# zju3dv/disprcnn

Hardware: AMD Instinct MI355X
Metric: ROI cost-volumes/sec (112x112x48) (higher is better)
Workload: dtype f32 (every convolution of the regressor, the three 32->1 heads included: split-f16 -- each fp32 value carried as hi + lo fp16, 3 f16-MFMA products per fp32 product, f32 accumulate; fp32-class error, tests/test_hip_s16.py.  Head gather and soft-argmin: f32 VALU); 1 GPU; Config A: per ROI pair, features [32,28,28]x2 -> concat cost volume [64,12,28,28] (folded into the first 3D layer's loads, never written) -> 3D stacked-hourglass regressor -> trilinear x4 + softmax + soft-argmin -> disparity [112,112]; maxdisp=48, mindisp=0, parallelism=roi-shard x1 (no collective), weights=closed-form synthetic (disprcnn_amd.utils.synth), BN stats calibrated fixture

## Files before the change

disprcnn_amd/_lib.py:

```python
import ctypes as C
import os

import torch

_HERE = os.path.dirname(os.path.abspath(__file__))
LIB_PATH = os.path.join(_HERE, "csrc", "libdisprcnn_hip.so")

DRC_MAX_CLASSES = 8


class DrcTapClass(C.Structure):
    _fields_ = [("nd", C.c_int32), ("nh", C.c_int32), ("nw", C.c_int32),
                ("dd0", C.c_int32), ("dh0", C.c_int32), ("dw0", C.c_int32),
                ("sd", C.c_int32), ("sh", C.c_int32), ("sw", C.c_int32),
                ("wbase", C.c_int32), ("wsd", C.c_int32), ("wsh", C.c_int32), ("wsw", C.c_int32),
                ("out_off_d", C.c_int32), ("out_off_h", C.c_int32), ("out_off_w", C.c_int32)]


class DrcTapconvParams(C.Structure):
    _fields_ = [("x", C.c_void_p), ("w", C.c_void_p), ("scale", C.c_void_p), ("shift", C.c_void_p),
                ("res", C.c_void_p), ("y", C.c_void_p),
                ("x_n_stride", C.c_int64), ("x_cb_stride", C.c_int64), ("x_d_stride", C.c_int64), ("x_h_stride", C.c_int64),
                ("y_n_stride", C.c_int64), ("y_cb_stride", C.c_int64), ("y_d_stride", C.c_int64), ("y_h_stride", C.c_int64),
                ("y_off0", C.c_int64),
                ("r_n_stride", C.c_int64), ("r_cb_stride", C.c_int64), ("r_d_stride", C.c_int64), ("r_h_stride", C.c_int64),
                ("r_off0", C.c_int64),
                ("N", C.c_int32), ("OD", C.c_int32), ("OH", C.c_int32), ("OW", C.c_int32),
                ("in_mul", C.c_int32), ("out_mul", C.c_int32), ("cb_in", C.c_int32), ("cout_pad", C.c_int32),
                ("R", C.c_int32), ("WT", C.c_int32), ("relu", C.c_int32), ("n_classes", C.c_int32),
                ("lds_bytes_per_wave", C.c_int32), ("reserved", C.c_int32),
                ("cls", DrcTapClass * DRC_MAX_CLASSES)]


class DrcCostvolSrc(C.Structure):
    _fields_ = [("left", C.c_void_p), ("right", C.c_void_p),
                ("n_stride", C.c_int64), ("cb_stride", C.c_int64), ("h_stride", C.c_int64),
                ("cbi", C.c_int32), ("pad", C.c_int32), ("lo4", C.c_int32), ("Wp", C.c_int32)]


class DrcS16ConvParams(C.Structure):
    _fields_ = [("x", C.c_void_p), ("w", C.c_void_p), ("scale", C.c_void_p), ("shift", C.c_void_p), ("res", C.c_void_p),
                ("y16", C.c_void_p), ("y32", C.c_void_p), ("left", C.c_void_p), ("right", C.c_void_p),
                ("N", C.c_int32), ("D", C.c_int32), ("H", C.c_int32), ("W", C.c_int32),
                ("cin", C.c_int32), ("cout", C.c_int32), ("relu", C.c_int32), ("lo4", C.c_int32), ("dil", C.c_int32),
                ("head", C.c_void_p), ("w1", C.c_void_p), ("ovf", C.c_void_p), ("head_rows", C.c_int32)]


class DrcFpnPyramid(C.Structure):
    _fields_ = [("feat", C.c_void_p * 8), ("H", C.c_int32 * 8), ("W", C.c_int32 * 8), ("scale", C.c_float * 8), ("n_levels", C.c_int32)]


class DrcSrpnLevels(C.Structure):
    _fields_ = [("n_levels", C.c_int32), ("N", C.c_int32), ("A", C.c_int32), ("C", C.c_int32), ("cap", C.c_int32), ("reserved", C.c_int32),
                ("H", C.c_int32 * 8), ("W", C.c_int32 * 8), ("pix_off", C.c_int64 * 9),
                ("left", C.c_void_p * 8), ("right", C.c_void_p * 8), ("hidden", C.c_void_p * 8), ("hidden_n_stride", C.c_int64 * 8),
                ("glogits", C.c_void_p * 8), ("gbbox", C.c_void_p * 8)]


class DrcWgradParams(C.Structure):
    _fields_ = [("a", C.c_void_p), ("b", C.c_void_p), ("gw", C.c_void_p),
                ("a_n_stride", C.c_int64), ("a_cb_stride", C.c_int64), ("a_d_stride", C.c_int64), ("a_h_stride", C.c_int64),
                ("b_n_stride", C.c_int64), ("b_cb_stride", C.c_int64), ("b_d_stride", C.c_int64), ("b_h_stride", C.c_int64),
                ("b_off0", C.c_int64),
                ("N", C.c_int32), ("OD", C.c_int32), ("OH", C.c_int32), ("OW", C.c_int32),
                ("in_mul", C.c_int32), ("cb_a", C.c_int32), ("cb_b", C.c_int32),
                ("nd", C.c_int32), ("nh", C.c_int32), ("nw", C.c_int32), ("dd0", C.c_int32), ("dh0", C.c_int32), ("dw0", C.c_int32),
                ("sd", C.c_int32), ("sh", C.c_int32), ("sw", C.c_int32),
                ("R", C.c_int32), ("WT", C.c_int32), ("lds_bytes_per_wave", C.c_int32), ("overwrite", C.c_int32),
                ("scratch", C.c_void_p), ("scratch_floats", C.c_int64)]


WGRAD_SCRATCH_FLOATS = (1024 + 3 * 64) * 49 * 256
LOSS_SCRATCH_FLOATS = 1024 * 8


def cout1_wgrad_scratch_floats(cb_in):
    return 1024 * cb_in * 27 * 16


_P = C.c_void_p
_I = C.c_int
_SIGS = {
    "drc_version": (C.c_char_p, []),
    "drc_cost_volume_fwd": (_I, [_P, _P, _P, _I, _I, _I, _I, _I, _I, _I, _P]),
    "drc_cost_volume_bwd": (_I, [_P, _P, _P, _I, _I, _I, _I, _I, _I, _I, _P]),
    "drc_cost_volume_blocked_fwd": (_I, [_P, _P, _P, _I, _I, _I, _I, _I, _I, _I, _I, _P]),
    "drc_dense_to_blocked": (_I, [_P, _P, _I, _I, _I, _I, _I, _I, _I, _I, _P]),
    "drc_blocked_to_dense": (_I, [_P, _P, _I, _I, _I, _I, _I, _I, _I, _I, _P]),
    "drc_tapconv_fwd": (_I, [C.POINTER(DrcTapconvParams), _P]),
    "drc_tapconv3d_direct_fwd": (_I, [C.POINTER(DrcTapconvParams), _I, _P]),
    "drc_deconv3d_k3s2_fwd": (_I, [C.POINTER(DrcTapconvParams), _P]),
    "drc_deconv3d_k3s2_direct_fwd": (_I, [C.POINTER(DrcTapconvParams), _I, _P]),
    "drc_conv3d_k3s2_direct_fwd": (_I, [C.POINTER(DrcTapconvParams), _I, _P]),
    "drc_conv3d_k3_wino_fwd": (_I, [C.POINTER(DrcTapconvParams), _I, _P]),
    "drc_linear_scratch_floats": (C.c_int64, [_I, _I, _I]),
    "drc_linear_packed_floats": (C.c_int64, [_I, _I]),
    "drc_linear_pack_rows": (_I, [_P, _I, _I, _P, _P]),
    "drc_linear_fwd": (_I, [_P, _P, _P, _P, _I, _I, _I, _I, _P, C.c_int64, _P]),
    "drc_linear_pack_cols": (_I, [_P, _I, _I, _P, _P]),
    "drc_relu_dropout_fwd": (_I, [_P, _P, _P, C.c_int64, C.c_float, _I, _P]),
    "drc_act_bwd_rows_scratch_doubles": (C.c_int64, [_I, _I]),
    "drc_act_bwd_rows": (_I, [_P, _P, _P, C.c_float, _I, _I, _I, _I, _P, _P, _P, C.c_int64, _P]),
    "drc_act_bwd_blocked_scratch_doubles": (C.c_int64, [_I, _I, _I]),
    "drc_act_bwd_blocked": (_I, [_P, _P, _I, _I, _I, _I, _I, _I, _I, _P, _P, _P, C.c_int64, _P]),
    "drc_roi_align_fpn_bwd": (_I, [C.POINTER(DrcFpnPyramid), _P, _P, _P, _I, _I, _I, _I, _I, _P]),
    "drc_srpn_active_pixels": (_I, [C.POINTER(DrcSrpnLevels), _P, _P, _P, _P, _P, _P]),
    "drc_srpn_gather_rows": (_I, [C.POINTER(DrcSrpnLevels), _P, _P, _P, _P, _P, _P, _P]),
    "drc_srpn_col2im": (_I, [C.POINTER(DrcSrpnLevels), _P, _P, _I, _P]),
    "drc_conv3d_k3_wino_rb_fwd": (_I, [C.POINTER(DrcTapconvParams), _P]),
    "drc_conv3d_k3_wino_rb_supported": (_I, [_I, _I, _I, _I]),
    "drc_conv2d_k3_wino_rb_supported": (_I, [_I, _I, _I]),
    "drc_conv2d_k3_wino_rb_fwd": (_I, [C.POINTER(DrcTapconvParams), _P]),
    "drc_pack_weights_wino2d_rb": (_I, [_P, _I, _I, _I, _I, _P, _P]),
    "drc_conv3d_k3_wino_rb_costvol_fwd": (_I, [C.POINTER(DrcTapconvParams), C.POINTER(DrcCostvolSrc), _P]),
    "drc_pack_weights_wino_rb": (_I, [_P, _I, _I, _I, _I, _P, _P]),
    "drc_box_decode_fwd": (_I, [_P, _P, _P, C.c_int64, _I, _I, _P, C.c_float, C.c_float, C.c_float, _P]),
    "drc_srpn_proposals_fwd": (_I, [_P, _P, _P, _P, _I, _I, _I, _I, C.c_int64, C.c_int64, C.c_float, _P, _P, _P, _P]),
    "drc_conv3d_k3_wino_costvol_fwd": (_I, [C.POINTER(DrcTapconvParams), C.POINTER(DrcCostvolSrc), _I, _P]),
    "drc_disparity_paste_fwd": (_I, [_P, _I, _P, _P, _I, _I, _I, _I, _P, _P, _P]),
    "drc_disparity_resize_fwd": (_I, [_P, _I, _I, _P, _I, _I, _I, _P]),
    "drc_roi_depth_maps_fwd": (_I, [_P, _I, _P, _P, _I, _I, _I, _P, _P]),
    "drc_conv2d_k3_wino_fwd": (_I, [C.POINTER(DrcTapconvParams), _I, _P]),
    "drc_pack_weights_wino2d": (_I, [_P, _I, _I, _I, _I, _P, _P]),
    "drc_pack_weights_wino": (_I, [_P, _I, _I, _I, _I, _P, _P]),
    "drc_conv2d_k1_fwd": (_I, [C.POINTER(DrcTapconvParams), _P]),
    "drc_conv2d_k3_direct_fwd": (_I, [C.POINTER(DrcTapconvParams), _I, _P]),
    "drc_conv3d_cout1_fwd": (_I, [_P, _P, _P, _P, _I, _I, _I, _I, _I, _P]),
    "drc_upsample_softargmin_fwd": (_I, [_P, _P, _I, _I, _I, _I, _I, _I, _I, _I, _P]),
    "drc_upsample_softargmin_form": (_I, [_I, _I, _I, _I, _I, _I]),
    "drc_avgpool2d_blocked": (_I, [_P, _P, _I, _I, _I, _I, _I, _I, _I, _I, _I, _P]),
    "drc_pack_weights": (_I, [_P, _I, _I, _I, _I, _I, _P, _P, _P]),
    "drc_avgpool2d_blocked_slice": (_I, [_P, _P, _I, _I, _I, _I, _I, _I, _I, _I, _I, _I, _I, _P]),
    "drc_bilinear_up_blocked": (_I, [_P, _P, _I, _I, _I, _I, _I, _I, _I, _I, _I, _I, _P]),
    "drc_bilinear_resize_blocked": (_I, [_P, _P, _I, _I, _I, _I, _I, _I, _I, _I, _I, _I, _I, _P]),
    "drc_maxpool2d_blocked": (_I, [_P, _P, _I, _I, _I, _I, _I, _I, _I, _I, _I, _I, _P]),
    "drc_copy_blocks": (_I, [_P, _P, _I, _I, C.c_int64, _I, _I, _P]),
    "drc_roi_align_fpn_fwd": (_I, [C.POINTER(DrcFpnPyramid), _P, _P, _P, _I, _I, _I, _I, _I, _P]),
    "drc_roi_align_fwd": (_I, [_P, _P, _P, _I, _I, _I, _I, _I, _I, C.c_float, _I, _P, _P, _P]),
    "drc_roi_align_bwd": (_I, [_P, _P, _P, _I, _I, _I, _I, _I, _I, C.c_float, _I, _P]),
    "drc_align_roi_pairs": (_I, [_P, _P, _P, _I, _I, _I, _P, _P, _P, _P]),
    "drc_conv16_fwd": (_I, [C.POINTER(DrcTapconvParams), _P]),
    "drc_dense_to_blocked16": (_I, [_P, _P, _I, _I, _I, _I, _I, _I, _P]),
    "drc_avgpool2d_blocked16_slice": (_I, [_P, _P, _I, _I, _I, _I, _I, _I, _I, _I, _I, _I, _I, _P]),
    "drc_bilinear_up_blocked16": (_I, [_P, _P, _I, _I, _I, _I, _I, _I, _I, _I, _I, _I, _P]),
    "drc_cost_volume16_from16": (_I, [_P, _P, _I, _I, _I, _I, _I, _I, _I, _I, _I, _P]),
    "drc_conv16_k3_tile_supported": (_I, [C.POINTER(DrcTapconvParams)]),
    "drc_conv16_k3_tile_fwd": (_I, [C.POINTER(DrcTapconvParams), _P]),
    "drc_conv2d_k3s2_stem_fwd": (_I, [_P, _I, _I, _I, _P, _I, _P, _P, _P, C.c_int64, C.c_int64, C.c_int64, C.c_int64, _I, _I, _I, _P]),
    "drc_conv16_k3_costvol_fwd": (_I, [C.POINTER(DrcTapconvParams), _I, _P]),
    "drc_conv16_k3s2_tile_supported": (_I, [C.POINTER(DrcTapconvParams)]),
    "drc_conv16_k3s2_tile_fwd": (_I, [C.POINTER(DrcTapconvParams), _P]),
    "drc_deconv16_k3s2_tile_supported": (_I, [C.POINTER(DrcTapconvParams)]),
    "drc_deconv16_k3s2_tile_fwd": (_I, [C.POINTER(DrcTapconvParams), _P]),
    "drc_cost_volume16_blocked_fwd": (_I, [_P, _P, _P, _I, _I, _I, _I, _I, _I, _I, _I, _P]),
    "drc_conv3d_k3_s16_supported": (_I, [_I, _I, _I, _I, _I]),
    "drc_conv3d_k3_s16_fwd": (_I, [C.POINTER(DrcS16ConvParams), _P]),
    "drc_conv3d_k3_s16_wide": (_I, [C.POINTER(DrcS16ConvParams)]),
    "drc_conv3d_k3_s16_wide_fwd": (_I, [C.POINTER(DrcS16ConvParams), _P]),
    "drc_conv3d_k3_s16_flat": (_I, [C.POINTER(DrcS16ConvParams)]),
    "drc_conv3d_k3s2_s16_supported": (_I, [_I, _I, _I, _I, _I]),
    "drc_conv3d_k3s2_s16_fwd": (_I, [C.POINTER(DrcS16ConvParams), _P]),
    "drc_deconv3d_k3s2_s16_supported": (_I, [_I, _I, _I, _I, _I]),
    "drc_deconv3d_k3s2_s16_fwd": (_I, [C.POINTER(DrcS16ConvParams), _P]),
    "drc_rs16_from_dense": (_I, [_P, _P, _I, _I, _I, _I, _I, _I, _P, _P]),
    "drc_rs16_from_blocked": (_I, [_P, _P, _I, _I, _I, _I, _I, _I, _I, _I, _I, _I, _I, _P, _P]),
    "drc_rs16_to_dense": (_I, [_P, _P, _I, _I, _I, _I, _I, _I, _P]),
    "drc_rs16_to_blocked": (_I, [_P, _P, _I, _I, _I, _I, _I, _I, _I, _I, _I, _I, _I, _P]),
    "drc_head_gather_fwd": (_I, [_P, _P, _P, _I, _I, _I, _I, C.c_float, _P]),
    "drc_head_gather_rows_fwd": (_I, [_P, _P, _P, C.c_float, C.c_float, C.c_float, _I, _P, _P, _I, _I, _I, _I, _P]),
    "drc_head_gather_planar_fwd": (_I, [_P, _P, _P, C.c_float, C.c_float, C.c_float, _I, _P, _P, _I, _I, _I, _I, _P]),
    "drc_conv2d_k3_s16_supported": (_I, [_I, _I, _I, _I, _I]),
    "drc_conv2d_k3_s16_fwd": (_I, [C.POINTER(DrcS16ConvParams), _P]),
    "drc_deconv3d_k3s2_direct_s16_fwd": (_I, [C.POINTER(DrcTapconvParams), _P, _P, _P]),
    "drc_nms_sorted_fwd": (_I, [_P, _I, C.c_float, _I, _P, _P, _P]),
    "drc_nms_sorted_batch_fwd": (_I, [_P, _I, _I, C.c_float, _I, _P, _P, _P]),
    "drc_nms_sorted_pair_joint_fwd": (_I, [_P, _I, C.c_float, _I, _I, _P, _P, _P]),
    "drc_roi_train_targets_fwd": (_I, [_P, _P, _P, _I, _I, C.c_float, _P, _P, _P, _I, _I, _I, _I, _P, _P, _P]),
    "drc_bn_stats_blocked": (_I, [_P, _P, _P, _P, _P]),
    "drc_bn_finalize": (_I, [_P, _I, _I, C.c_longlong, C.c_float, C.c_float, _P, _P, _P, _P, _P]),
    "drc_bn_apply_blocked": (_I, [_P, _P, _P, _P, _P, _P, _P, _P, _P, _P, _I, _P]),
    "drc_tapconv_wgrad": (_I, [C.POINTER(DrcWgradParams), _P]),
    "drc_bilinear_up_blocked_bwd": (_I, [_P, _P, _P, _P, _P]),
    "drc_avgpool2d_blocked_bwd": (_I, [_P, _P, _P, _P, _I, _P]),
    "drc_upsample_softargmin_bwd_scratch_floats": (C.c_int64, [_I, _I, _I, _I, _I, _I]),
    "drc_upsample_softargmin_bwd": (_I, [_P, _P, _P, _I, _I, _I, _I, _I, _I, _I, _I, _P, C.c_int64, _P]),
    "drc_conv3d_cout1_bwd_data": (_I, [_P, _P, _P, _I, _I, _I, _I, _I, _I, _P]),
    "drc_conv3d_cout1_bwd_weight": (_I, [_P, _P, _P, _I, _I, _I, _I, _I, _P, _P]),
    "drc_bn_bwd_reduce": (_I, [_P, _P, _P, _P, _P, _P, _P, _P, _I, _P, _P, _P]),
    "drc_bn_bwd_apply": (_I, [_P, _P, _P, _P, _P, _P, _P, _P, _P, _P, C.c_float, _I, _P, _P, _P, _P, _I, _P]),
    "drc_psm_loss_sums": (_I, [_P, _P, _P, _P, _P, C.c_int64, _P, _P, _P]),
    "drc_psm_loss_grad": (_I, [_P, _P, _P, C.c_int64, _P, C.c_float, _P, _P, _P]),
}

EXPORTED_SYMBOLS = tuple(_SIGS)

_lib = None


def lib():
    global _lib
    if _lib is None:
        if not os.path.exists(LIB_PATH):
            raise RuntimeError(
                f"{LIB_PATH} is missing: the HIP extension is not built. Run "
                "`python -c 'import __graft_entry__ as g; g.build()'` (or python -m disprcnn_amd.csrc.build). "
                "There is no CPU/torch fallback for this path.")
        handle = C.CDLL(LIB_PATH)
        for name, (res, args) in _SIGS.items():
            fn = getattr(handle, name)
            fn.restype = res
            fn.argtypes = args
        _lib = handle
    return _lib


def check(status, what):
    if status != 0:
        kind = "bad argument / unsupported shape" if status < 0 else "hipError_t"
        raise RuntimeError(f"{what} failed: status {status} ({kind})")
```

disprcnn_amd/csrc/build.py:

```python
import os
import subprocess
import sys

HERE = os.path.dirname(os.path.abspath(__file__))
SOURCES = ["tapconv.hip", "tapdirect.hip", "wino3d.hip", "wino3d_rb.hip", "wino2d.hip", "tapdeconv.hip", "deconvdirect.hip", "downdirect.hip", "stemconv.hip", "pointwise.hip", "linear.hip", "head_train.hip", "srpn_train.hip", "volume_ops.hip", "cout1_mfma.hip", "roi_ops.hip", "nms_ops.hip", "det_ops.hip", "post_ops.hip", "train_ops.hip", "bwd_ops.hip", "wgrad.hip", "wgrad_slide.hip", "conv16.hip", "conv16t.hip", "conv16x.hip", "ops16.hip", "convs16.hip", "convs16w.hip", "convs16d.hip", "convs16u.hip", "convs16r.hip", "s16_ops.hip"]
LIB = os.path.join(HERE, "libdisprcnn_hip.so")
HIPCC = os.environ.get("HIPCC", "/opt/rocm/bin/hipcc")
FLAGS = ["--offload-arch=gfx950", "-O3", "-std=c++17", "-fPIC", "-ffp-contract=off", "-Wall", "-Wno-unused-function", "-Wno-pass-failed"]


def _sources():
    return [os.path.join(HERE, s) for s in SOURCES if os.path.exists(os.path.join(HERE, s))]


def _headers():
    return [os.path.join(HERE, "..", "..", "include", "disprcnn_hip.h")] + \
        [os.path.join(HERE, f) for f in sorted(os.listdir(HERE)) if f.endswith(".h")]


def source_digest():
    import hashlib
    h = hashlib.sha256()
    for f in sorted(_sources() + _headers(), key=os.path.basename):
        h.update(os.path.basename(f).encode())
        h.update(open(f, "rb").read())
    return h.hexdigest()[:16]


def needs_build():
    if not os.path.exists(LIB):
        return True
    t = os.path.getmtime(LIB)
    return any(os.path.getmtime(d) > t for d in _sources() + _headers())


def build(force=False, verbose=True):
    if not force and not needs_build():
        return LIB
    objs, jobs = [], []
    for src in _sources():
        obj = src[:-4] + ".o"
        if force or not os.path.exists(obj) or os.path.getmtime(obj) < max(os.path.getmtime(d) for d in [src] + _headers()):
            jobs.append([HIPCC] + FLAGS + ["-c", src, "-o", obj])
        objs.append(obj)
    if jobs:
        from concurrent.futures import ThreadPoolExecutor

        def run(cmd):
            if verbose:
                print(" ".join(cmd), flush=True)
            subprocess.check_call(cmd)
        with ThreadPoolExecutor(max_workers=max(1, min(len(jobs), os.cpu_count() or 1))) as ex:
            list(ex.map(run, jobs))
    cmd = [HIPCC, "--offload-arch=gfx950", "-shared", "-fPIC", "-o", LIB] + objs
    if verbose:
        print(" ".join(cmd), flush=True)
    subprocess.check_call(cmd)
    return LIB


if __name__ == "__main__":
    build(force="--force" in sys.argv)
    print(LIB)
```

disprcnn_amd/csrc/s16_ops.hip:

```cpp
#include <hip/hip_runtime.h>
#include <stdint.h>

#include "../../include/disprcnn_hip.h"
#include "s16_ovf.h"

typedef float f32x4 __attribute__((ext_vector_type(4)));
typedef _Float16 f16x8 __attribute__((ext_vector_type(8)));

namespace {

__device__ inline void split8(const float (&v)[8], f16x8& hi, f16x8& lo, S16Ovf& og) {
#pragma unroll
    for (int e = 0; e < 8; ++e) {
        og.see_raw(v[e]);
        float x = fminf(fmaxf(v[e], -65504.f), 65504.f);
        hi[e] = (_Float16)x;
        lo[e] = (_Float16)(x - (float)hi[e]);
    }
}

__global__ void rs16_from_dense_kernel(const float* __restrict__ x, _Float16* __restrict__ y, int N, int C, int D, int H, int W, int pd, uint32_t* ovf) {
    S16Ovf og;
    const long total = (long)N * (C / 32) * D * H * 4 * W;
    const int Wp = W + 2, Hp = H + 2, Dp = D + 2 * pd;
    for (long i = (long)blockIdx.x * blockDim.x + threadIdx.x; i < total; i += (long)gridDim.x * blockDim.x) {
        long t = i;
        const int xw = (int)(t % W); t /= W;
        const int sg = (int)(t % 4); t /= 4;
        const int yh = (int)(t % H); t /= H;
        const int z = (int)(t % D); t /= D;
        const int cb = (int)(t % (C / 32));
        const int n = (int)(t / (C / 32));
        const int s = sg >> 1, g = sg & 1;
        float v[8];
#pragma unroll
        for (int e = 0; e < 8; ++e) {
            const int c = cb * 32 + 4 * g + 8 * (2 * s + (e >> 2)) + (e & 3);
            v[e] = x[((((long)n * C + c) * D + z) * H + yh) * W + xw];
        }
        f16x8 hi, lo;
        split8(v, hi, lo, og);
        _Float16* row = y + (((((long)n * (C / 32) + cb) * Dp + z + pd) * Hp + yh + 1) * 8) * (long)Wp * 8;
        *(f16x8*)(row + ((long)sg * Wp + xw + 1) * 8) = hi;
        *(f16x8*)(row + ((long)(4 + sg) * Wp + xw + 1) * 8) = lo;
    }
    og.flush(ovf);
}

__global__ void rs16_from_blocked_kernel(const float* __restrict__ x, _Float16* __restrict__ y, int N, int C, int D, int H, int W, int pdi, int phi,
                                         int pwi, int cb16_total, int cb16_off, int pd, uint32_t* ovf) {
    S16Ovf og;
    const long total = (long)N * (C / 32) * D * H * 4 * W;
    const int Wp = W + 2, Hp = H + 2, Dp = D + 2 * pd;
    const long xw_ = W + 2 * pwi, xh_ = H + 2 * phi, xd_ = D + 2 * pdi;
    for (long i = (long)blockIdx.x * blockDim.x + threadIdx.x; i < total; i += (long)gridDim.x * blockDim.x) {
        long t = i;
        const int sg = (int)(t % 4); t /= 4;
        const int xw = (int)(t % W); t /= W;
        const int yh = (int)(t % H); t /= H;
        const int z = (int)(t % D); t /= D;
        const int cb = (int)(t % (C / 32));
        const int n = (int)(t / (C / 32));
        const int s = sg >> 1, g = sg & 1;
        const float* src = x + (((((long)n * cb16_total + cb16_off + 2 * cb + s) * xd_ + z + pdi) * xh_ + yh + phi) * xw_ + xw + pwi) * 16 + 4 * g;
        const f32x4 a = *(const f32x4*)src, b = *(const f32x4*)(src + 8);
        const float v[8] = {a.x, a.y, a.z, a.w, b.x, b.y, b.z, b.w};
        f16x8 hi, lo;
        split8(v, hi, lo, og);
        _Float16* row = y + (((((long)n * (C / 32) + cb) * Dp + z + pd) * Hp + yh + 1) * 8) * (long)Wp * 8;
        *(f16x8*)(row + ((long)sg * Wp + xw + 1) * 8) = hi;
        *(f16x8*)(row + ((long)(4 + sg) * Wp + xw + 1) * 8) = lo;
    }
    og.flush(ovf);
}

__global__ void rs16_to_dense_kernel(const _Float16* __restrict__ y, float* __restrict__ x, int N, int C, int D, int H, int W, int pd) {
    const long total = (long)N * (C / 32) * D * H * 4 * W;
    const int Wp = W + 2, Hp = H + 2, Dp = D + 2 * pd;
    for (long i = (long)blockIdx.x * blockDim.x + threadIdx.x; i < total; i += (long)gridDim.x * blockDim.x) {
        long t = i;
        const int xw = (int)(t % W); t /= W;
        const int sg = (int)(t % 4); t /= 4;
        const int yh = (int)(t % H); t /= H;
        const int z = (int)(t % D); t /= D;
        const int cb = (int)(t % (C / 32));
        const int n = (int)(t / (C / 32));
        const int s = sg >> 1, g = sg & 1;
        const _Float16* row = y + (((((long)n * (C / 32) + cb) * Dp + z + pd) * Hp + yh + 1) * 8) * (long)Wp * 8;
        const f16x8 hi = *(const f16x8*)(row + ((long)sg * Wp + xw + 1) * 8);
        const f16x8 lo = *(const f16x8*)(row + ((long)(4 + sg) * Wp + xw + 1) * 8);
#pragma unroll
        for (int e = 0; e < 8; ++e) {
            const int c = cb * 32 + 4 * g + 8 * (2 * s + (e >> 2)) + (e & 3);
            x[((((long)n * C + c) * D + z) * H + yh) * W + xw] = (float)hi[e] + (float)lo[e];
        }
    }
}

__global__ void rs16_to_blocked_kernel(const _Float16* __restrict__ y, float* __restrict__ x, int N, int C, int D, int H, int W, int pdo, int pho,
                                       int pwo, int cb16_total, int cb16_off, int pd) {
    const long total = (long)N * (C / 32) * D * H * 4 * W;
    const int Wp = W + 2, Hp = H + 2, Dp = D + 2 * pd;
    const long xw_ = W + 2 * pwo, xh_ = H + 2 * pho, xd_ = D + 2 * pdo;
    for (long i = (long)blockIdx.x * blockDim.x + threadIdx.x; i < total; i += (long)gridDim.x * blockDim.x) {
        long t = i;
        const int sg = (int)(t % 4); t /= 4;
        const int xw = (int)(t % W); t /= W;
        const int yh = (int)(t % H); t /= H;
        const int z = (int)(t % D); t /= D;
        const int cb = (int)(t % (C / 32));
        const int n = (int)(t / (C / 32));
        const int s = sg >> 1, g = sg & 1;
        const _Float16* row = y + (((((long)n * (C / 32) + cb) * Dp + z + pd) * Hp + yh + 1) * 8) * (long)Wp * 8;
        const f16x8 hi = *(const f16x8*)(row + ((long)sg * Wp + xw + 1) * 8);
        const f16x8 lo = *(const f16x8*)(row + ((long)(4 + sg) * Wp + xw + 1) * 8);
        float* dst = x + (((((long)n * cb16_total + cb16_off + 2 * cb + s) * xd_ + z + pdo) * xh_ + yh + pho) * xw_ + xw + pwo) * 16 + 4 * g;
        *(f32x4*)dst = (f32x4){(float)hi[0] + (float)lo[0], (float)hi[1] + (float)lo[1], (float)hi[2] + (float)lo[2], (float)hi[3] + (float)lo[3]};
        *(f32x4*)(dst + 8) = (f32x4){(float)hi[4] + (float)lo[4], (float)hi[5] + (float)lo[5], (float)hi[6] + (float)lo[6], (float)hi[7] + (float)lo[7]};
    }
}

inline unsigned grid_for(long total) {
    long b = (total + 255) / 256;
    return (unsigned)(b < 1 ? 1 : (b > 256 * 32 ? 256 * 32 : b));
}

}

extern "C" int drc_rs16_from_dense(const float* x, void* y16, int N, int C, int D, int H, int W, int pd, uint32_t* ovf, void* stream) {
    if (!x || !y16) return -1;
    if (N < 0 || C <= 0 || (C & 31) || D <= 0 || H <= 0 || W <= 0 || pd < 0 || pd > 1) return -2;
    if (N == 0) return 0;
    hipLaunchKernelGGL(rs16_from_dense_kernel, dim3(grid_for((long)N * (C / 32) * D * H * 4 * W)), dim3(256), 0, (hipStream_t)stream, x, (_Float16*)y16, N, C, D, H, W, pd, ovf);
    return (int)hipGetLastError();
}

extern "C" int drc_rs16_from_blocked(const float* xb, void* y16, int N, int C, int D, int H, int W, int pd_in, int ph_in, int pw_in, int cb16_total,
                                     int cb16_off, int pd, uint32_t* ovf, void* stream) {
    if (!xb || !y16) return -1;
    if (N < 0 || C <= 0 || (C & 31) || D <= 0 || H <= 0 || W <= 0 || pd < 0 || pd > 1 || pd_in < 0 || ph_in < 0 || pw_in < 0 || cb16_off < 0 ||
        cb16_off + C / 16 > cb16_total)
        return -2;
    if (N == 0) return 0;
    hipLaunchKernelGGL(rs16_from_blocked_kernel, dim3(grid_for((long)N * (C / 32) * D * H * 4 * W)), dim3(256), 0, (hipStream_t)stream, xb, (_Float16*)y16, N, C, D,
                       H, W, pd_in, ph_in, pw_in, cb16_total, cb16_off, pd, ovf);
    return (int)hipGetLastError();
}

extern "C" int drc_rs16_to_dense(const void* y16, float* x, int N, int C, int D, int H, int W, int pd, void* stream) {
    if (!x || !y16) return -1;
    if (N < 0 || C <= 0 || (C & 31) || D <= 0 || H <= 0 || W <= 0 || pd < 0 || pd > 1) return -2;
    if (N == 0) return 0;
    hipLaunchKernelGGL(rs16_to_dense_kernel, dim3(grid_for((long)N * (C / 32) * D * H * 4 * W)), dim3(256), 0, (hipStream_t)stream, (const _Float16*)y16, x, N, C, D, H, W, pd);
    return (int)hipGetLastError();
}

extern "C" int drc_rs16_to_blocked(const void* y16, float* xb, int N, int C, int D, int H, int W, int pd_out, int ph_out, int pw_out, int cb16_total,
                                   int cb16_off, int pd, void* stream) {
    if (!xb || !y16) return -1;
    if (N < 0 || C <= 0 || (C & 31) || D <= 0 || H <= 0 || W <= 0 || pd < 0 || pd > 1 || pd_out < 0 || ph_out < 0 || pw_out < 0 || cb16_off < 0 ||
        cb16_off + C / 16 > cb16_total)
        return -2;
    if (N == 0) return 0;
    hipLaunchKernelGGL(rs16_to_blocked_kernel, dim3(grid_for((long)N * (C / 32) * D * H * 4 * W)), dim3(256), 0, (hipStream_t)stream, (const _Float16*)y16, xb, N, C,
                       D, H, W, pd_out, ph_out, pw_out, cb16_total, cb16_off, pd);
    return (int)hipGetLastError();
}

namespace {
__global__ __launch_bounds__(256) void head_gather_kernel(const float* __restrict__ S, const float* __restrict__ res, float* __restrict__ cost,
                                                          long total, int H, int W, float scale) {
    const long i = (long)blockIdx.x * 256 + threadIdx.x;
    if (i >= total) return;
    const int x = (int)(i % W);
    const long row = i / W;
    const int y = (int)(row % H);
    float a = 0.f;
#pragma unroll
    for (int kh = 0; kh < 3; ++kh) {
        const int yy = y + kh - 1;
        if (yy < 0 || yy >= H) continue;
        const float* sr = S + ((row + (kh - 1)) * W) * 12;
#pragma unroll
        for (int kw = 0; kw < 3; ++kw) {
            const int xx = x + kw - 1;
            if (xx < 0 || xx >= W) continue;
            const int j = kh * 3 + kw;
            a += sr[(long)xx * 12 + (j < 5 ? j : j + 3)];
        }
    }
    a *= scale;
    cost[i] = res ? a + res[i] : a;
}
}

namespace {
__global__ __launch_bounds__(256) void head_gather_lds_kernel(const float* __restrict__ S, const float* __restrict__ res, float* __restrict__ cost,
                                                              int H, int W, int R, int bands, float scale) {
    extern __shared__ __attribute__((aligned(16))) float tile[];
    typedef float f32x4 __attribute__((ext_vector_type(4)));
    const long plane = blockIdx.x / bands;
    const int y0 = (int)(blockIdx.x % bands) * R;
    const int rows = H - y0 < R ? H - y0 : R;
    const int Wt = W + 2, nt = (rows + 2) * Wt;
    const float* sp = S + plane * (long)H * W * 12;
    for (int i = threadIdx.x; i < nt; i += 256) {
        const int ry = i / Wt, rx = i - ry * Wt;
        const int y = y0 - 1 + ry, x = rx - 1;
        f32x4 a = {0.f, 0.f, 0.f, 0.f}, b = a, c = a;
        if (y >= 0 && y < H && x >= 0 && x < W) {
            const f32x4* q = (const f32x4*)(sp + ((long)y * W + x) * 12);
            a = q[0]; b = q[1]; c = q[2];
        }
        float* t = tile + i * 9;
        t[0] = a[0]; t[1] = a[1]; t[2] = a[2]; t[3] = a[3]; t[4] = b[0];
        t[5] = c[0]; t[6] = c[1]; t[7] = c[2]; t[8] = c[3];
    }
    __syncthreads();
    const int no = rows * W;
    const long o0 = (plane * H + y0) * (long)W;
    for (int i = threadIdx.x; i < no; i += 256) {
        const int ry = i / W, rx = i - ry * W;
        float v = 0.f;
#pragma unroll
        for (int kh = 0; kh < 3; ++kh)
#pragma unroll
            for (int kw = 0; kw < 3; ++kw) v += tile[((ry + kh) * Wt + rx + kw) * 9 + kh * 3 + kw];
        v *= scale;
        cost[o0 + i] = res ? v + res[o0 + i] : v;
    }
}
}

extern "C" int drc_head_gather_fwd(const float* S, const float* res, float* cost, int N, int D, int H, int W, float scale, void* stream) {
    if (!S || !cost) return -1;
    if (N < 0 || D <= 0 || H <= 0 || W <= 0) return -2;
    if (N == 0) return 0;
    const long total = (long)N * D * H * W;
    const long per_row = (long)(W + 2) * 36;
    long R = 40960 / per_row - 2;
    if (R >= 1) {
        if (R > H) R = H;
        const long bands = (H + R - 1) / R;
        const long blocks = (long)N * D * bands;
        if (blocks > 0x7fffffffL) return -3;
        hipLaunchKernelGGL(head_gather_lds_kernel, dim3((unsigned)blocks), dim3(256), (size_t)((R + 2) * per_row), (hipStream_t)stream, S, res, cost, H, W,
                           (int)R, (int)bands, scale);
        return (int)hipGetLastError();
    }
    const long blocks = (total + 255) / 256;
    if (blocks > 0x7fffffffL) return -3;
    hipLaunchKernelGGL(head_gather_kernel, dim3((unsigned)blocks), dim3(256), 0, (hipStream_t)stream, S, res, cost, total, H, W, scale);
    return (int)hipGetLastError();
}

namespace {
struct HeadRows {
    const float* rows[3];
    float scale[3];
};
template <int NH>
__global__ __launch_bounds__(256) void head_gather_rows_kernel(const HeadRows hr, const float* __restrict__ res, float* __restrict__ cost, long cols, int H, int W) {
    typedef float f32x4 __attribute__((ext_vector_type(4)));
    const long i = (long)blockIdx.x * 256 + threadIdx.x;
    if (i >= cols) return;
    const long plane = i / W;
    const long base = plane * H * W + (i - plane * W);
    const f32x4* r[NH];
    f32x4 cur[NH];
    float up[NH];
#pragma unroll
    for (int k = 0; k < NH; ++k) {
        r[k] = (const f32x4*)hr.rows[k] + base;
        cur[k] = r[k][0];
        up[k] = 0.f;
    }
    for (int y0 = 0; y0 < H; y0 += 4) {
        f32x4 nx[4][NH];
        float rs[4];
#pragma unroll
        for (int j = 0; j < 4; ++j) {
            const int yn = y0 + j + 1 < H ? y0 + j + 1 : H - 1, yr = y0 + j < H ? y0 + j : H - 1;
#pragma unroll
            for (int k = 0; k < NH; ++k) nx[j][k] = r[k][(long)yn * W];
            rs[j] = res ? res[base + (long)yr * W] : 0.f;
        }
#pragma unroll
        for (int j = 0; j < 4; ++j) {
            const int y = y0 + j;
            if (y < H) {
                float c = rs[j];
#pragma unroll
                for (int k = 0; k < NH; ++k) {
                    float s = up[k] + (cur[k][1] + cur[k][2]);
                    if (y + 1 < H) s += nx[j][k][3];
                    c = hr.scale[k] * s + c;
                }
                cost[base + (long)y * W] = c;
            }
#pragma unroll
            for (int k = 0; k < NH; ++k) {
                up[k] = cur[k][0];
                cur[k] = nx[j][k];
            }
        }
    }
}
template <int NH>
__global__ __launch_bounds__(256) void head_gather_planar_kernel(const HeadRows hr, const float* __restrict__ res, float* __restrict__ cost, long total, int H, int W) {
    const long i = (long)blockIdx.x * 256 + threadIdx.x;
    if (i >= total) return;
    const long HW = (long)H * W;
    const long plane = i / HW;
    const int e = (int)(i - plane * HW);
    const int y = e / W, x = e - y * W;
    const bool xm = x > 0, xp = x + 1 < W, ym = y > 0, yp = y + 1 < H;
    const int dm = xm ? -1 : 0, dp = xp ? 1 : 0, du = ym ? -W : 0, dd = yp ? W : 0;
    float v[NH][9];
#pragma unroll
    for (int k = 0; k < NH; ++k) {
        const float* p = hr.rows[k] + plane * 9 * HW + e;
#pragma unroll
        for (int j = 0; j < 9; ++j) v[k][j] = p[j * HW + (j < 3 ? du : j < 6 ? 0 : dd) + (j % 3 == 0 ? dm : j % 3 == 2 ? dp : 0)];
    }
    float c = res ? res[i] : 0.f;
#pragma unroll
    for (int k = 0; k < NH; ++k) {
        const float* q = v[k];
        const float l0 = xm ? q[0] : 0.f, l3 = xm ? q[3] : 0.f, l6 = xm ? q[6] : 0.f;
        const float r2 = xp ? q[2] : 0.f, r5 = xp ? q[5] : 0.f, r8 = xp ? q[8] : 0.f;
        const float t0 = (l0 + q[1]) + r2;
        const float t1a = l3 + q[4];
        const float t1b = r5;
        const float t2 = (l6 + q[7]) + r8;
        float s = (ym ? t0 : 0.f) + (t1a + t1b);
        if (yp) s += t2;
        c = hr.scale[k] * s + c;
    }
    cost[i] = c;
}
}

extern "C" int drc_head_gather_planar_fwd(const float* s0, const float* s1, const float* s2, float scale0, float scale1, float scale2, int nheads,
                                          const float* res, float* cost, int N, int D, int H, int W, void* stream) {
    if (nheads < 1 || nheads > 3) return -2;
    const HeadRows hr = {{s0, s1, s2}, {scale0, scale1, scale2}};
    for (int k = 0; k < nheads; ++k)
        if (!hr.rows[k] || ((uintptr_t)hr.rows[k] & 3)) return -1;
    if (!cost) return -1;
    if (N < 0 || D <= 0 || H <= 0 || W <= 0) return -2;
    if (N == 0) return 0;
    const long cols = (long)N * D * H * W;
    const long blocks = (cols + 255) / 256;
    if (blocks > 0x7fffffffL) return -3;
    const dim3 g((unsigned)blocks), b(256);
    hipStream_t s = (hipStream_t)stream;
    if (nheads == 1) hipLaunchKernelGGL(head_gather_planar_kernel<1>, g, b, 0, s, hr, res, cost, cols, H, W);
    else if (nheads == 2) hipLaunchKernelGGL(head_gather_planar_kernel<2>, g, b, 0, s, hr, res, cost, cols, H, W);
    else hipLaunchKernelGGL(head_gather_planar_kernel<3>, g, b, 0, s, hr, res, cost, cols, H, W);
    return (int)hipGetLastError();
}

extern "C" int drc_head_gather_rows_fwd(const float* rows0, const float* rows1, const float* rows2, float scale0, float scale1, float scale2, int nheads,
                                        const float* res, float* cost, int N, int D, int H, int W, void* stream) {
    if (nheads < 1 || nheads > 3) return -2;
    const HeadRows hr = {{rows0, rows1, rows2}, {scale0, scale1, scale2}};
    for (int k = 0; k < nheads; ++k)
        if (!hr.rows[k] || ((uintptr_t)hr.rows[k] & 15)) return -1;
    if (!cost) return -1;
    if (N < 0 || D <= 0 || H <= 0 || W <= 0) return -2;
    if (N == 0) return 0;
    const long cols = (long)N * D * W;
    const long blocks = (cols + 255) / 256;
    if (blocks > 0x7fffffffL) return -3;
    const dim3 g((unsigned)blocks), b(256);
    hipStream_t s = (hipStream_t)stream;
    if (nheads == 1) hipLaunchKernelGGL(head_gather_rows_kernel<1>, g, b, 0, s, hr, res, cost, cols, H, W);
    else if (nheads == 2) hipLaunchKernelGGL(head_gather_rows_kernel<2>, g, b, 0, s, hr, res, cost, cols, H, W);
    else hipLaunchKernelGGL(head_gather_rows_kernel<3>, g, b, 0, s, hr, res, cost, cols, H, W);
    return (int)hipGetLastError();
}
```

disprcnn_amd/csrc/volume_ops.hip:

```cpp
#include <hip/hip_runtime.h>
#include <stdint.h>

#include "../../include/disprcnn_hip.h"

typedef float f32x4 __attribute__((ext_vector_type(4)));

namespace {

constexpr int kThreads = 256;

inline unsigned grid_for(long work, int cap = 256 * 16) {
    long b = (work + kThreads - 1) / kThreads;
    if (b < 1) b = 1;
    if (b > cap) b = cap;
    return (unsigned)b;
}

template <bool VEC4>
__global__ __launch_bounds__(kThreads) void cost_volume_dense_kernel(const float* __restrict__ L, const float* __restrict__ R,
                                                                     float* __restrict__ cost, int N, int C, int Dp, int Hp, int Wp,
                                                                     int lo4, int hi4) {
    const int XV = VEC4 ? 4 : 1;
    const int wq = Wp / XV;
    const long total = (long)N * 2 * C * Dp * Hp * wq;
    for (long idx = (long)blockIdx.x * kThreads + threadIdx.x; idx < total; idx += (long)gridDim.x * kThreads) {
        long t = idx;
        const int xq = (int)(t % wq); t /= wq;
        const int y = (int)(t % Hp); t /= Hp;
        const int j = (int)(t % Dp); t /= Dp;
        const int c2 = (int)(t % (2 * C));
        const int n = (int)(t / (2 * C));
        const int i = lo4 + j;
        const bool live = i < hi4;
        const int x0 = xq * XV;
        float v[4];
        const bool right = c2 >= C;
        const int c = right ? c2 - C : c2;
        const float* src = (right ? R : L) + (((long)n * C + c) * Hp + y) * Wp;
#pragma unroll
        for (int e = 0; e < XV; ++e) {
            const int x = x0 + e, xs = x - i;
            const bool ok = live && xs >= 0 && xs < Wp;
            v[e] = ok ? src[right ? xs : x] : 0.0f;
        }
        float* dst = cost + ((((long)n * 2 * C + c2) * Dp + j) * Hp + y) * Wp + x0;
        if (VEC4) *(f32x4*)dst = (f32x4){v[0], v[1], v[2], v[3]};
        else dst[0] = v[0];
    }
}

__global__ __launch_bounds__(kThreads) void cost_volume_bwd_kernel(const float* __restrict__ g, float* __restrict__ gL,
                                                                   float* __restrict__ gR, int N, int C, int Dp, int Hp, int Wp,
                                                                   int lo4, int hi4) {
    const long per = (long)N * C * Hp * Wp;
    for (long idx = (long)blockIdx.x * kThreads + threadIdx.x; idx < 2 * per; idx += (long)gridDim.x * kThreads) {
        const bool right = idx >= per;
        long t = right ? idx - per : idx;
        const int x = (int)(t % Wp); t /= Wp;
        const int y = (int)(t % Hp); t /= Hp;
        const int c = (int)(t % C);
        const int n = (int)(t / C);
        float s = 0.f;
        for (int j = 0; j < Dp; ++j) {
            const int i = lo4 + j;
            if (i >= hi4) break;
            const int xo = right ? x + i : x;
            const int xs = xo - i;
            const bool ok = right ? (xo >= 0 && xo < Wp) : (xs >= 0 && xs < Wp);
            if (ok) s += g[((((long)n * 2 * C + (right ? C + c : c)) * Dp + j) * Hp + y) * Wp + xo];
        }
        (right ? gR : gL)[(((long)n * C + c) * Hp + y) * Wp + x] = s;
    }
}

__global__ __launch_bounds__(kThreads) void cost_volume_blocked_kernel(const float* __restrict__ L, const float* __restrict__ R,
                                                                       float* __restrict__ out, int N, int C, int Dp, int Hp, int Wp,
                                                                       int lo4, int hi4, int fp) {
    const int CBo = 2 * C / 16, CBi = C / 16;
    const long total = (long)N * CBo * Dp * Hp * Wp * 4;
    const long oH = Wp + 2, oD = (long)(Hp + 2) * oH, oC = (long)(Dp + 2) * oD;
    for (long idx = (long)blockIdx.x * kThreads + threadIdx.x; idx < total; idx += (long)gridDim.x * kThreads) {
        long t = idx;
        const int q = (int)(t & 3); t >>= 2;
        const int x = (int)(t % Wp); t /= Wp;
        const int y = (int)(t % Hp); t /= Hp;
        const int j = (int)(t % Dp); t /= Dp;
        const int cbo = (int)(t % CBo);
        const int n = (int)(t / CBo);
        const int i = lo4 + j;
        const int xs = x - i;
        const bool ok = (i < hi4) && xs >= 0 && xs < Wp;
        const bool right = cbo >= CBi;
        const int cbi = right ? cbo - CBi : cbo;
        const int xr = right ? xs : x;
        f32x4 v = {0.f, 0.f, 0.f, 0.f};
        if (ok) {
            const float* src = right ? R : L;
            if (fp > 0) {
                const long iW = Wp + 2 * fp, iH = Hp + 2 * fp;
                v = *(const f32x4*)(src + ((((long)n * CBi + cbi) * iH + (y + fp)) * iW + (xr + fp)) * 16 + q * 4);
            } else {
                const long plane = (long)Hp * Wp;
                const float* s0 = src + ((long)n * C + cbi * 16 + q * 4) * plane + (long)y * Wp + xr;
                v = (f32x4){s0[0], s0[plane], s0[2 * plane], s0[3 * plane]};
            }
        }
        *(f32x4*)(out + (((long)n * CBo + cbo) * oC + (long)(j + 1) * oD + (long)(y + 1) * oH + (x + 1)) * 16 + q * 4) = v;
    }
}


__global__ __launch_bounds__(kThreads) void cost_volume_blocked_rows_kernel(const float* __restrict__ L, const float* __restrict__ R,
                                                                            float* __restrict__ out, int C, int Dp, int Hp, int Wp, int lo4, int hi4) {
    extern __shared__ float cv_lds[];
    const int n = blockIdx.x / Hp, y = blockIdx.x - n * Hp;
    const int cs = C + 1;
    float* lL = cv_lds;
    float* lR = cv_lds + (long)Wp * cs;
    const long plane = (long)Hp * Wp;
    const int xl = threadIdx.x & 31, sub = threadIdx.x >> 5, nsub = kThreads >> 5;
    for (int c = sub; c < 2 * C; c += nsub) {
        const bool right = c >= C;
        const int cc = right ? c - C : c;
        const float* src = (right ? R : L) + ((long)n * C + cc) * plane + (long)y * Wp;
        float* dst = right ? lR : lL;
        for (int x = xl; x < Wp; x += 32) dst[x * cs + cc] = src[x];
    }
    __syncthreads();
    const int CBi = C / 16, CBo = 2 * CBi;
    const long oH = Wp + 2, oD = (long)(Hp + 2) * oH, oC = (long)(Dp + 2) * oD;
    const int per_row = Wp * 4;
    const int total = CBo * Dp * per_row;
    for (int idx = threadIdx.x; idx < total; idx += kThreads) {
        int t = idx;
        const int q = t & 3; t >>= 2;
        const int x = t % Wp; t /= Wp;
        const int j = t % Dp;
        const int cbo = t / Dp;
        const int i = lo4 + j;
        const int xs = x - i;
        const bool ok = (i < hi4) && xs >= 0 && xs < Wp;
        const bool right = cbo >= CBi;
        f32x4 v = {0.f, 0.f, 0.f, 0.f};
        if (ok) {
            const float* s = (right ? lR + xs * cs + (cbo - CBi) * 16 : lL + x * cs + cbo * 16) + q * 4;
            v = (f32x4){s[0], s[1], s[2], s[3]};
        }
        *(f32x4*)(out + (((long)n * CBo + cbo) * oC + (long)(j + 1) * oD + (long)(y + 1) * oH + (x + 1)) * 16 + q * 4) = v;
    }
}

__global__ __launch_bounds__(kThreads) void dense_to_blocked_kernel(const float* __restrict__ dense, float* __restrict__ blk, int N, int C,
                                                                    int D, int H, int W, int pd, int ph, int pw) {
    const int CB = (C + 15) / 16;
    const long total = (long)N * CB * D * H * W * 4;
    const long bW = W + 2 * pw, bH = H + 2 * ph, bD = D + 2 * pd;
// ... 85 lines not shown
#pragma unroll
                for (int kh = 0; kh < 3; ++kh)
#pragma unroll
                    for (int kw = 0; kw < 3; ++kw) {
                        const f32x4 xv = *(const f32x4*)(xb + cb * sC + kd * sD + kh * sH + kw * 16);
                        const f32x4 wv = *(const f32x4*)(w + ((kd * 3 + kh) * 3 + kw) * cb_in * 16 + cb * 16 + q * 4);
                        s = fmaf(xv.x, wv.x, s); s = fmaf(xv.y, wv.y, s); s = fmaf(xv.z, wv.z, s); s = fmaf(xv.w, wv.w, s);
                    }
        }
        s += __shfl_xor(s, 1);
        s += __shfl_xor(s, 2);
        if (live && q == 0) out[vox] = res ? s + res[vox] : s;
    }
}


#define GLOBAL_PTR(p) ((const __attribute__((address_space(1))) void*)(p))
#define LDS_PTR(p) ((__attribute__((address_space(3))) void*)(p))
constexpr int kC1Waves = 4;
__global__ __launch_bounds__(64 * kC1Waves) void conv3d_cout1_slide_kernel(const float* __restrict__ x, const float* __restrict__ w,
                                                                           const float* __restrict__ res, float* __restrict__ out, int N,
                                                                           int cb_in, int D, int H, int W, int R, int seg_len) {
    extern __shared__ __attribute__((aligned(16))) float lds_c1[];
    const int wave = __builtin_amdgcn_readfirstlane(threadIdx.x >> 6);
    const int lane = threadIdx.x & 63;
    const int n_rt = (H + R - 1) / R;
    int cid = blockIdx.x * kC1Waves + wave;
    if (cid >= N * n_rt) return;
    const int rt = cid % n_rt, n = cid / n_rt;
    const int oh0 = rt * R;
    const int Wp = W + 2, Hp = H + 2;
    const long sH = (long)Wp * 16, sD = (long)Hp * sH, sC = (long)(D + 2) * sD, sN = sC * cb_in;
    const int rows_in = R + 2;
    const int seg_floats = Wp * 16, seg_units = Wp * 4;
    const int buf_floats = rows_in * seg_floats;
    float* lds = lds_c1 + wave * 2 * buf_floats;
    const float* xcol = x + n * sN + (long)oh0 * sH;
    const int nvox = R * W;
    int voff[2]; bool vok[2]; int vr[2], vc[2];
#pragma unroll
    for (int k = 0; k < 2; ++k) {
        const int s = lane + 64 * k;
        vok[k] = s < nvox && oh0 + s / W < H;
        vr[k] = vok[k] ? s / W : 0; vc[k] = vok[k] ? s - (s / W) * W : 0;
        voff[k] = (vr[k] * Wp + vc[k]) * 16;
    }
    auto stage = [&](int d_in, int cb, int bufi) {
        const float* src = xcol + cb * sC + (long)(d_in + 1) * sD;
        float* dst = lds + bufi * buf_floats;
        for (int r = 0; r < rows_in; ++r)
            for (int u0 = 0; u0 < seg_units; u0 += 64) {
                const int u = u0 + lane;
                if (u < seg_units) __builtin_amdgcn_global_load_lds(GLOBAL_PTR(src + r * sH + u * 4), LDS_PTR(dst + r * seg_floats + u0 * 4), 16, 0, 0);
            }
    };
    float a0[2] = {0.f, 0.f}, a1[2] = {0.f, 0.f}, a2[2] = {0.f, 0.f};
    const int od_lo = blockIdx.y * seg_len;
    const int od_hi = od_lo + seg_len < D ? od_lo + seg_len : D;
    const int din_lo = od_lo > 0 ? od_lo - 1 : 0, din_hi = od_hi < D ? od_hi : D - 1;
    int bufsel = 0;
    stage(din_lo, 0, 0);
    asm volatile("s_waitcnt vmcnt(0)" ::: "memory");
    const int rot = lane & 3;
    for (int d_in = din_lo; d_in <= din_hi; ++d_in) {
        const bool v0 = d_in + 1 < D;
        const bool v2 = d_in - 1 >= od_lo && d_in - 1 < od_hi;
        const bool v1s = d_in + 1 == D && d_in >= od_lo;
        for (int cb = 0; cb < cb_in; ++cb) {
            const bool last = cb + 1 == cb_in;
            if (!last || d_in + 1 <= din_hi) stage(last ? d_in + 1 : d_in, last ? 0 : cb + 1, bufsel ^ 1);
            const float* buf = lds + bufsel * buf_floats;
#pragma unroll
            for (int kh = 0; kh < 3; ++kh)
#pragma unroll
                for (int kw = 0; kw < 3; ++kw) {
                    const int t = kh * 3 + kw;
                    const float* w0 = w + ((0 * 9 + t) * cb_in + cb) * 16;
                    const float* w1 = w + ((1 * 9 + t) * cb_in + cb) * 16;
                    const float* w2 = w + ((2 * 9 + t) * cb_in + cb) * 16;
#pragma unroll
                    for (int k = 0; k < 2; ++k) {
                        const float* px = buf + voff[k] + (kh * Wp + kw) * 16;
#pragma unroll
                        for (int qq = 0; qq < 4; ++qq) {
                            const int q = (qq + rot) & 3;
                            const f32x4 v = *(const f32x4*)(px + q * 4);
                            const f32x4 u0 = *(const f32x4*)(w0 + q * 4), u1 = *(const f32x4*)(w1 + q * 4), u2 = *(const f32x4*)(w2 + q * 4);
                            a0[k] = fmaf(v.x, u0.x, fmaf(v.y, u0.y, fmaf(v.z, u0.z, fmaf(v.w, u0.w, a0[k]))));
                            a1[k] = fmaf(v.x, u1.x, fmaf(v.y, u1.y, fmaf(v.z, u1.z, fmaf(v.w, u1.w, a1[k]))));
                            a2[k] = fmaf(v.x, u2.x, fmaf(v.y, u2.y, fmaf(v.z, u2.z, fmaf(v.w, u2.w, a2[k]))));
                        }
                    }
                }
            asm volatile("s_waitcnt vmcnt(0)" ::: "memory");
            bufsel ^= 1;
        }
#pragma unroll
        for (int k = 0; k < 2; ++k) {
            const long o = (((long)n * D) * H + (oh0 + vr[k])) * W + vc[k];
            if (vok[k] && v2) { const long oo = o + (long)(d_in - 1) * H * W; out[oo] = res ? a2[k] + res[oo] : a2[k]; }
            if (vok[k] && v1s) { const long oo = o + (long)d_in * H * W; out[oo] = res ? a1[k] + res[oo] : a1[k]; }
            a2[k] = a1[k]; a1[k] = v0 ? a0[k] : 0.f; a0[k] = 0.f;
        }
    }
}

constexpr int kSAThreads = 128;
__global__ __launch_bounds__(kSAThreads) void upsample_softargmin_kernel(const float* __restrict__ cost, float* __restrict__ disp, int N,
                                                                         int Dp, int Hp, int Wp, int D, int H, int W, int mindisp) {
    extern __shared__ float cz[];
    const long total = (long)N * H * W;
    const long idx = (long)blockIdx.x * kSAThreads + threadIdx.x;
    if (idx >= total) return;
    long t = idx;
    const int x = (int)(t % W); t /= W;
    const int y = (int)(t % H);
    const int n = (int)(t / H);
    const float sy = H > 1 ? (float)(Hp - 1) / (float)(H - 1) : 0.f;
    const float sx = W > 1 ? (float)(Wp - 1) / (float)(W - 1) : 0.f;
    const float sd = D > 1 ? (float)(Dp - 1) / (float)(D - 1) : 0.f;
    const float fy = sy * y, fx = sx * x;
    const int y0 = (int)fy, x0 = (int)fx;
    const int y1 = y0 + (y0 < Hp - 1), x1 = x0 + (x0 < Wp - 1);
    const float ty = fy - y0, tx = fx - x0;
    const float* c = cost + (long)n * Dp * Hp * Wp;
    for (int k = 0; k < Dp; ++k) {
        const float* s = c + (long)k * Hp * Wp;
        const float a = s[y0 * Wp + x0] * (1.f - tx) + s[y0 * Wp + x1] * tx;
        const float b = s[y1 * Wp + x0] * (1.f - tx) + s[y1 * Wp + x1] * tx;
        cz[k * kSAThreads + threadIdx.x] = a * (1.f - ty) + b * ty;
    }
    float m = -INFINITY;
    for (int d = 0; d < D; ++d) {
        const float fd = sd * d;
        const int k0 = (int)fd;
        const int k1 = k0 + (k0 < Dp - 1);
        const float td = fd - k0;
        m = fmaxf(m, cz[k0 * kSAThreads + threadIdx.x] * (1.f - td) + cz[k1 * kSAThreads + threadIdx.x] * td);
    }
    float se = 0.f, sde = 0.f;
    for (int d = 0; d < D; ++d) {
        const float fd = sd * d;
        const int k0 = (int)fd;
        const int k1 = k0 + (k0 < Dp - 1);
        const float td = fd - k0;
        const float v = cz[k0 * kSAThreads + threadIdx.x] * (1.f - td) + cz[k1 * kSAThreads + threadIdx.x] * td;
        const float e = expf(v - m);
        se += e;
        sde = fmaf(e, (float)(mindisp + d), sde);
    }
    disp[idx] = sde / se;
}

template <int DP, int D>
__global__ __launch_bounds__(256) void upsample_softargmin_t_kernel(const float* __restrict__ cost, float* __restrict__ disp, int N, int Hp, int Wp,
                                                                    int H, int W, int mindisp, int blocks_per_roi) {
    extern __shared__ float rows[];
    int b = blockIdx.x;
    if ((gridDim.x & 7) == 0) b = (b & 7) * (gridDim.x >> 3) + (b >> 3);
    const int n = b / blocks_per_roi;
    const int pix0 = (b - n * blocks_per_roi) * 256;
    const int HW = H * W;
    const int pl = pix0 + 255 < HW ? pix0 + 255 : HW - 1;
    const float sy = H > 1 ? (float)(Hp - 1) / (float)(H - 1) : 0.f;
    const float sx = W > 1 ? (float)(Wp - 1) / (float)(W - 1) : 0.f;
    const int cy0 = (int)(sy * (pix0 / W));
    int cy1 = (int)(sy * (pl / W)) + 1;
    cy1 = cy1 > Hp - 1 ? Hp - 1 : cy1;
    const int nrows = cy1 - cy0 + 1;
    const float* c = cost + (long)n * DP * Hp * Wp;
    const int lpr = Wp <= 32 ? 32 : 64, xl = (int)threadIdx.x & (lpr - 1);
    for (int rk = (int)threadIdx.x / lpr; rk < nrows * DP; rk += 256 / lpr) {
        const int r = rk / DP, k = rk - r * DP;
        if (xl < Wp) rows[rk * Wp + xl] = c[((long)k * Hp + cy0 + r) * Wp + xl];
    }
    __syncthreads();
    const int pix = pix0 + (int)threadIdx.x;
    if (pix >= HW) return;
    const int y = pix / W, x = pix - y * W;
    const float fy = sy * y, fx = sx * x;
    const int y0 = (int)fy, x0 = (int)fx;
    const int y1 = y0 + (y0 < Hp - 1), x1 = x0 + (x0 < Wp - 1);
    const float ty = fy - y0, tx = fx - x0;
    const float* r0 = rows + (y0 - cy0) * DP * Wp;
    const float* r1 = rows + (y1 - cy0) * DP * Wp;
    float cz[DP];
#pragma unroll
    for (int k = 0; k < DP; ++k) {
        const float a = r0[k * Wp + x0] * (1.f - tx) + r0[k * Wp + x1] * tx;
        const float bb = r1[k * Wp + x0] * (1.f - tx) + r1[k * Wp + x1] * tx;
        cz[k] = a * (1.f - ty) + bb * ty;
    }
    constexpr float sd = D > 1 ? (float)(DP - 1) / (float)(D - 1) : 0.f;
    float v[D];
    float m = -INFINITY;
#pragma unroll
    for (int d = 0; d < D; ++d) {
        constexpr float dummy = 0.f; (void)dummy;
        const float fd = sd * (float)d;
        const int k0 = (int)fd;
        const int k1 = k0 + (k0 < DP - 1);
        const float td = fd - (float)k0;
        v[d] = cz[k0] * (1.f - td) + cz[k1] * td;
        m = fmaxf(m, v[d]);
    }
    float se = 0.f, sde = 0.f;
#pragma unroll
    for (int d = 0; d < D; ++d) {
        const float e = __builtin_amdgcn_exp2f((v[d] - m) * 1.44269504088896340736f);
        se += e;
        sde = fmaf(e, (float)(mindisp + d), sde);
    }
    disp[(long)n * HW + pix] = sde / se;
}

template <int DP, int D>
static int launch_softargmin_t(const float* cost, float* disp, int N, int Hp, int Wp, int H, int W, int mindisp, hipStream_t stream) {
    const int bpr = (H * W + 255) / 256;
    const long blocks = (long)N * bpr;
    hipLaunchKernelGGL((upsample_softargmin_t_kernel<DP, D>), dim3((unsigned)blocks), dim3(256), (size_t)3 * DP * Wp * sizeof(float), stream, cost, disp, N,
                       Hp, Wp, H, W, mindisp, bpr);
    return (int)hipGetLastError();
}

__global__ __launch_bounds__(64) void avgpool2d_blocked_kernel(const float* __restrict__ x, float* __restrict__ y, int N, int CB, int H,
                                                               int W, int px, int k, int OH, int OW, int py, int x_cb_total, int x_cb_off) {
    long t = blockIdx.x;
    const int ow = (int)(t % OW); t /= OW;
    const int oh = (int)(t % OH); t /= OH;
    const int cb = (int)(t % CB);
    const int n = (int)(t / CB);
    const int lane = threadIdx.x, q = lane & 3, p0 = lane >> 2;
    const long iW = W + 2 * px, iH = H + 2 * px;
    const float* xb = x + (((long)n * x_cb_total + x_cb_off + cb) * iH + (oh * k + px)) * iW * 16 + (long)(ow * k + px) * 16 + q * 4;
    f32x4 s = {0.f, 0.f, 0.f, 0.f};
    for (int p = p0; p < k * k; p += 16) {
        const int r = p / k, c = p - r * k;
        s += *(const f32x4*)(xb + ((long)r * iW + c) * 16);
    }
#pragma unroll
    for (int m = 4; m < 64; m <<= 1) {
        s.x += __shfl_xor(s.x, m); s.y += __shfl_xor(s.y, m); s.z += __shfl_xor(s.z, m); s.w += __shfl_xor(s.w, m);
    }
    if (p0 == 0) {
        const float inv = 1.0f / (float)(k * k);
        const long oW = OW + 2 * py, oH = OH + 2 * py;
        *(f32x4*)(y + ((((long)n * CB + cb) * oH + (oh + py)) * oW + (ow + py)) * 16 + q * 4) = s * inv;
    }
}

__global__ __launch_bounds__(kThreads) void bilinear_up_blocked_kernel(const float* __restrict__ x, float* __restrict__ y, int N, int CB,
                                                                       int IH, int IW, int px, int OH, int OW, int py, int y_cb_total,
                                                                       int y_cb_off, int align_corners) {
    const long total = (long)N * CB * OH * OW * 4;
    const long iW = IW + 2 * px, iH = IH + 2 * px, oW = OW + 2 * py, oH = OH + 2 * py;
    const float sy = align_corners ? (OH > 1 ? (float)(IH - 1) / (float)(OH - 1) : 0.f) : (float)IH / (float)OH;
    const float sx = align_corners ? (OW > 1 ? (float)(IW - 1) / (float)(OW - 1) : 0.f) : (float)IW / (float)OW;
    for (long idx = (long)blockIdx.x * kThreads + threadIdx.x; idx < total; idx += (long)gridDim.x * kThreads) {
        long t = idx;
        const int q = (int)(t & 3); t >>= 2;
        const int ox = (int)(t % OW); t /= OW;
        const int oy = (int)(t % OH); t /= OH;
        const int cb = (int)(t % CB);
        const int n = (int)(t / CB);
        const float fy = align_corners ? sy * oy : fmaxf(sy * (oy + 0.5f) - 0.5f, 0.f);
        const float fx = align_corners ? sx * ox : fmaxf(sx * (ox + 0.5f) - 0.5f, 0.f);
        const int y0 = (int)fy, x0 = (int)fx;
        const int y1 = y0 + (y0 < IH - 1), x1 = x0 + (x0 < IW - 1);
        const float ty = fy - y0, tx = fx - x0;
        const float* xb = x + (((long)n * CB + cb) * iH) * iW * 16 + q * 4;
        const f32x4 v00 = *(const f32x4*)(xb + ((long)(y0 + px) * iW + (x0 + px)) * 16);
        const f32x4 v01 = *(const f32x4*)(xb + ((long)(y0 + px) * iW + (x1 + px)) * 16);
        const f32x4 v10 = *(const f32x4*)(xb + ((long)(y1 + px) * iW + (x0 + px)) * 16);
        const f32x4 v11 = *(const f32x4*)(xb + ((long)(y1 + px) * iW + (x1 + px)) * 16);
        const f32x4 v = (1.f - ty) * ((1.f - tx) * v00 + tx * v01) + ty * ((1.f - tx) * v10 + tx * v11);
        *(f32x4*)(y + ((((long)n * y_cb_total + y_cb_off + cb) * oH + (oy + py)) * oW + (ox + py)) * 16 + q * 4) = v;
    }
}

__global__ __launch_bounds__(kThreads) void maxpool2d_blocked_kernel(const float* __restrict__ x, float* __restrict__ y, int N, int CB, int H,
                                                                     int W, int px, int k, int stride, int OH, int OW, int py) {
    const long total = (long)N * CB * OH * OW * 4;
    const long iW = W + 2 * px, iH = H + 2 * px, oW = OW + 2 * py, oH = OH + 2 * py;
    for (long idx = (long)blockIdx.x * kThreads + threadIdx.x; idx < total; idx += (long)gridDim.x * kThreads) {
        long t = idx;
        const int q = (int)(t & 3); t >>= 2;
        const int ox = (int)(t % OW); t /= OW;
        const int oy = (int)(t % OH); t /= OH;
        const int cb = (int)(t % CB);
        const int n = (int)(t / CB);
        const float* xb = x + (((long)n * CB + cb) * iH) * iW * 16 + q * 4;
        f32x4 m = {-INFINITY, -INFINITY, -INFINITY, -INFINITY};
        for (int a = 0; a < k; ++a) {
            const int iy = oy * stride + a;
            if (iy >= H) break;
            for (int b = 0; b < k; ++b) {
                const int ix = ox * stride + b;
                if (ix >= W) break;
                const f32x4 v = *(const f32x4*)(xb + ((long)(iy + px) * iW + (ix + px)) * 16);
                m.x = fmaxf(m.x, v.x); m.y = fmaxf(m.y, v.y); m.z = fmaxf(m.z, v.z); m.w = fmaxf(m.w, v.w);
            }
        }
        *(f32x4*)(y + ((((long)n * CB + cb) * oH + (oy + py)) * oW + (ox + py)) * 16 + q * 4) = m;
    }
}

__global__ __launch_bounds__(kThreads) void copy_blocks_kernel(const float* __restrict__ x, float* __restrict__ y, int N, int CB,
                                                               long vox_per_cb, int y_cb_total, int y_cb_off) {
    const long per = vox_per_cb * 4;
    const long total = (long)N * CB * per;
    for (long idx = (long)blockIdx.x * kThreads + threadIdx.x; idx < total; idx += (long)gridDim.x * kThreads) {
        const long e = idx % per;
        long t = idx / per;
        const int cb = (int)(t % CB);
        const int n = (int)(t / CB);
        *(f32x4*)(y + (((long)n * y_cb_total + y_cb_off + cb) * per + e) * 4) = *(const f32x4*)(x + idx * 4);
    }
}

inline int done() { return (int)hipGetLastError(); }

}

__global__ __launch_bounds__(256) void pack_weights_kernel(const float* __restrict__ w, int cout, int cin, int K, int transposed, int flip,
                                                           float* __restrict__ out_tap, float* __restrict__ out_t16) {
    const int cb_n = (cin + 15) / 16, cout_pad = (cout + 15) / 16 * 16;
    const long total = (long)K * cb_n * cout_pad * 16;
    for (long idx = (long)blockIdx.x * 256 + threadIdx.x; idx < total; idx += (long)gridDim.x * 256) {
        long t = idx;
        const int c = (int)(t & 15); t >>= 4;
        const int co = (int)(t % cout_pad); t /= cout_pad;
        const int cb = (int)(t % cb_n);
        const int k = (int)(t / cb_n);
        const int ci = cb * 16 + c;
        float v = 0.f;
        if (co < cout && ci < cin) {
            const int ks = flip ? K - 1 - k : k;
            v = transposed ? w[((long)ci * cout + co) * K + ks] : w[((long)co * cin + ci) * K + ks];
        }
        if (out_t16) out_t16[idx] = v;
        if (out_tap) out_tap[((((long)k * cb_n + cb) * 2 + (c >> 3)) * cout_pad + co) * 8 + (c & 7)] = v;
    }
}

extern "C" int drc_conv3d_cout1_mfma_try(const float* x, const float* w, const float* res, float* out, int N, int cb_in, int D, int H, int W,
                                         void* stream);

extern "C" {

const char* drc_version(void) { return "disprcnn_hip gfx950 abi1"; }

int drc_cost_volume_fwd(const float* left, const float* right, float* cost, int N, int C, int Dp, int Hp, int Wp, int lo4, int hi4,
                        void* stream) {
    if (N < 0 || C <= 0 || Dp < 0 || Hp <= 0 || Wp <= 0) return -2;
    const long total = (long)N * 2 * C * Dp * Hp * Wp;
    if (total == 0) return 0;
    if (!left || !right || !cost) return -1;
    hipStream_t s = (hipStream_t)stream;
    if (Wp % 4 == 0 && ((uintptr_t)cost & 15) == 0)
        hipLaunchKernelGGL(cost_volume_dense_kernel<true>, dim3(grid_for(total / 4)), dim3(kThreads), 0, s, left, right, cost, N, C, Dp, Hp, Wp, lo4, hi4);
    else
        hipLaunchKernelGGL(cost_volume_dense_kernel<false>, dim3(grid_for(total)), dim3(kThreads), 0, s, left, right, cost, N, C, Dp, Hp, Wp, lo4, hi4);
    return done();
}

int drc_cost_volume_bwd(const float* gcost, float* gleft, float* gright, int N, int C, int Dp, int Hp, int Wp, int lo4, int hi4,
                        void* stream) {
    if (N < 0 || C <= 0 || Dp < 0 || Hp <= 0 || Wp <= 0) return -2;
    const long total = 2L * N * C * Hp * Wp;
    if (total == 0) return 0;
    if (!gcost || !gleft || !gright) return -1;
    hipLaunchKernelGGL(cost_volume_bwd_kernel, dim3(grid_for(total)), dim3(kThreads), 0, (hipStream_t)stream, gcost, gleft, gright, N, C, Dp, Hp, Wp, lo4, hi4);
    return done();
}

int drc_cost_volume_blocked_fwd(const float* left, const float* right, float* cost_blk, int N, int C, int Dp, int Hp, int Wp, int lo4,
                                int hi4, int in_blocked_pad, void* stream) {
    if (N < 0 || C <= 0 || (C & 15) || Dp < 0 || Hp <= 0 || Wp <= 0 || in_blocked_pad < 0) return -2;
    const long total = (long)N * (2 * C / 16) * Dp * Hp * Wp * 4;
    if (total == 0) return 0;
    if (!left || !right || !cost_blk) return -1;
    const size_t lds = (size_t)2 * Wp * (C + 1) * sizeof(float);
    if (in_blocked_pad == 0 && lds <= 64 * 1024 && (long)N * Hp < (1L << 31)) {
        hipLaunchKernelGGL(cost_volume_blocked_rows_kernel, dim3((unsigned)(N * Hp)), dim3(kThreads), lds, (hipStream_t)stream, left, right, cost_blk, C,
                           Dp, Hp, Wp, lo4, hi4);
        return done();
    }
    hipLaunchKernelGGL(cost_volume_blocked_kernel, dim3(grid_for(total)), dim3(kThreads), 0, (hipStream_t)stream, left, right, cost_blk, N, C, Dp, Hp, Wp, lo4, hi4, in_blocked_pad);
    return done();
}

int drc_dense_to_blocked(const float* dense, float* blk, int N, int C, int D, int H, int W, int pd, int ph, int pw, void* stream) {
    if (N < 0 || C <= 0 || D <= 0 || H <= 0 || W <= 0 || pd < 0 || ph < 0 || pw < 0) return -2;
    const long total = (long)N * ((C + 15) / 16) * D * H * W * 4;
    if (total == 0) return 0;
    if (!dense || !blk) return -1;
    const size_t lds = (size_t)W * (((C + 15) / 16) * 16 + 1) * sizeof(float);
    const long lines = (long)N * D * H;
    if (W >= 8 && lds <= 64 * 1024 && lines < (1L << 31))
        hipLaunchKernelGGL(dense_to_blocked_rows_kernel, dim3((unsigned)lines), dim3(kThreads), lds, (hipStream_t)stream, dense, blk, C, D, H, W, pd, ph, pw);
    else
        hipLaunchKernelGGL(dense_to_blocked_kernel, dim3(grid_for(total)), dim3(kThreads), 0, (hipStream_t)stream, dense, blk, N, C, D, H, W, pd, ph, pw);
    return done();
}

int drc_blocked_to_dense(const float* blk, float* dense, int N, int C, int D, int H, int W, int pd, int ph, int pw, void* stream) {
    if (N < 0 || C <= 0 || D <= 0 || H <= 0 || W <= 0 || pd < 0 || ph < 0 || pw < 0) return -2;
    const long total = (long)N * C * D * H * W;
    if (total == 0) return 0;
    if (!dense || !blk) return -1;
    hipLaunchKernelGGL(blocked_to_dense_kernel, dim3(grid_for(total)), dim3(kThreads), 0, (hipStream_t)stream, blk, dense, N, C, D, H, W, pd, ph, pw);
    return done();
}

int drc_conv3d_cout1_fwd(const float* x, const float* w, const float* res, float* out, int N, int cb_in, int D, int H, int W,
                         void* stream) {
    if (N < 0 || cb_in <= 0 || D <= 0 || H <= 0 || W <= 0) return -2;
    const long total = (long)N * D * H * W * 4;
    if (total == 0) return 0;
    if (!x || !w || !out) return -1;
    {
        const int st = drc_conv3d_cout1_mfma_try(x, w, res, out, N, cb_in, D, H, W, stream);
        if (st != 1) return st;
    }
    int R = 128 / (W > 0 ? W : 1);
    if (R > H) R = H;
    while (R > 1 && H % R && (H + R - 1) / R * R - H > R / 2) --R;
    const size_t lds = R >= 1 ? (size_t)kC1Waves * 2 * (R + 2) * (W + 2) * 64 : 0;
    if (W <= 64 && R >= 1 && lds <= 160 * 1024 && D >= 2) {
        static bool attr_done = false;
        if (!attr_done) {
            (void)hipFuncSetAttribute((const void*)conv3d_cout1_slide_kernel, hipFuncAttributeMaxDynamicSharedMemorySize, 160 * 1024);
            attr_done = true;
        }
        const long cols = (long)N * ((H + R - 1) / R);
        int nseg = (int)(1024 / (cols > 0 ? cols : 1));
        if (nseg > D / 3) nseg = D / 3;
        if (nseg < 1) nseg = 1;
        const int seg_len = (D + nseg - 1) / nseg;
        nseg = (D + seg_len - 1) / seg_len;
        hipLaunchKernelGGL(conv3d_cout1_slide_kernel, dim3((unsigned)((cols + kC1Waves - 1) / kC1Waves), (unsigned)nseg), dim3(64 * kC1Waves), lds,
                           (hipStream_t)stream, x, w, res, out, N, cb_in, D, H, W, R, seg_len);
        return done();
    }
    hipLaunchKernelGGL(conv3d_cout1_kernel, dim3(grid_for(total, 256 * 32)), dim3(kThreads), 0, (hipStream_t)stream, x, w, res, out, N, cb_in, D, H, W);
    return done();
}

int drc_upsample_softargmin_form(int Dp, int Hp, int Wp, int D, int H, int W) {
    if (Dp <= 0 || Hp <= 0 || Wp <= 0 || D <= 0 || H <= 0 || W <= 0) return -2;
    if (Dp > 96) return -3;
    if (D == 4 * Dp && H > 1 && W >= 86 && Wp <= 64 && (size_t)3 * Dp * Wp * 4 <= 64 * 1024) {
        const float sy = (float)(Hp - 1) / (float)(H - 1);
        if (sy * (float)((255 + W - 1) / W) < 1.f && (Dp == 6 || Dp == 12 || Dp == 24)) return Dp;
    }
    return 0;
}

int drc_upsample_softargmin_fwd(const float* cost, float* disp, int N, int Dp, int Hp, int Wp, int D, int H, int W, int mindisp,
                                void* stream) {
    if (N < 0) return -2;
    int form = drc_upsample_softargmin_form(Dp, Hp, Wp, D, H, W);
    if (form < 0) return form;
    const long total = (long)N * H * W;
    if (total == 0) return 0;
    if (!cost || !disp) return -1;
    if ((long)N * ((H * W + 255) / 256) >= (1L << 31)) form = 0;
    hipStream_t s = (hipStream_t)stream;
    if (form == 12) return launch_softargmin_t<12, 48>(cost, disp, N, Hp, Wp, H, W, mindisp, s);
    if (form == 24) return launch_softargmin_t<24, 96>(cost, disp, N, Hp, Wp, H, W, mindisp, s);
    if (form == 6) return launch_softargmin_t<6, 24>(cost, disp, N, Hp, Wp, H, W, mindisp, s);
    const unsigned blocks = (unsigned)((total + kSAThreads - 1) / kSAThreads);
    hipLaunchKernelGGL(upsample_softargmin_kernel, dim3(blocks), dim3(kSAThreads), (size_t)Dp * kSAThreads * 4, (hipStream_t)stream, cost, disp, N, Dp, Hp, Wp, D, H, W, mindisp);
    return done();
}

int drc_avgpool2d_blocked(const float* x, float* y, int N, int CB, int H, int W, int px, int k, int OH, int OW, int py, void* stream) {
    if (N < 0 || CB <= 0 || H <= 0 || W <= 0 || k <= 0 || OH <= 0 || OW <= 0 || OH * k > H || OW * k > W) return -2;
    const long blocks = (long)N * CB * OH * OW;
    if (blocks == 0) return 0;
    if (!x || !y) return -1;
    hipLaunchKernelGGL(avgpool2d_blocked_kernel, dim3((unsigned)blocks), dim3(64), 0, (hipStream_t)stream, x, y, N, CB, H, W, px, k, OH, OW, py, CB, 0);
    return done();
}

int drc_pack_weights(const float* w, int cout, int cin, int K, int transposed, int flip, float* out_tap, float* out_t16, void* stream) {
    if (cout <= 0 || cin <= 0 || K <= 0) return -2;
    if (!w || (!out_tap && !out_t16)) return -1;
    const long total = (long)K * ((cin + 15) / 16) * ((cout + 15) / 16 * 16) * 16;
    hipLaunchKernelGGL(pack_weights_kernel, dim3(grid_for(total, 2048)), dim3(256), 0, (hipStream_t)stream, w, cout, cin, K, transposed, flip,
                       out_tap, out_t16);
    return done();
}

int drc_avgpool2d_blocked_slice(const float* x, float* y, int N, int CB, int H, int W, int px, int k, int OH, int OW, int py, int x_cb_total,
                                int x_cb_off, void* stream) {
    if (N < 0 || CB <= 0 || H <= 0 || W <= 0 || k <= 0 || OH <= 0 || OW <= 0 || OH * k > H || OW * k > W) return -2;
    if (x_cb_off < 0 || x_cb_off + CB > x_cb_total) return -2;
    const long blocks = (long)N * CB * OH * OW;
    if (blocks == 0) return 0;
    if (!x || !y) return -1;
    hipLaunchKernelGGL(avgpool2d_blocked_kernel, dim3((unsigned)blocks), dim3(64), 0, (hipStream_t)stream, x, y, N, CB, H, W, px, k, OH, OW, py,
                       x_cb_total, x_cb_off);
    return done();
}

int drc_bilinear_up_blocked(const float* x, float* y, int N, int CB, int IH, int IW, int px, int OH, int OW, int py, int y_cb_total,
                            int y_cb_off, void* stream) {
    if (N < 0 || CB <= 0 || IH <= 0 || IW <= 0 || OH <= 0 || OW <= 0 || y_cb_off < 0 || y_cb_off + CB > y_cb_total) return -2;
    const long total = (long)N * CB * OH * OW * 4;
    if (total == 0) return 0;
    if (!x || !y) return -1;
    hipLaunchKernelGGL(bilinear_up_blocked_kernel, dim3(grid_for(total)), dim3(kThreads), 0, (hipStream_t)stream, x, y, N, CB, IH, IW, px, OH, OW, py, y_cb_total, y_cb_off, 1);
    return done();
}

int drc_bilinear_resize_blocked(const float* x, float* y, int N, int CB, int IH, int IW, int px, int OH, int OW, int py, int y_cb_total,
                                int y_cb_off, int align_corners, void* stream) {
    if (N < 0 || CB <= 0 || IH <= 0 || IW <= 0 || OH <= 0 || OW <= 0 || y_cb_off < 0 || y_cb_off + CB > y_cb_total) return -2;
    const long total = (long)N * CB * OH * OW * 4;
    if (total == 0) return 0;
    if (!x || !y) return -1;
    hipLaunchKernelGGL(bilinear_up_blocked_kernel, dim3(grid_for(total)), dim3(kThreads), 0, (hipStream_t)stream, x, y, N, CB, IH, IW, px, OH, OW, py, y_cb_total, y_cb_off, align_corners ? 1 : 0);
    return done();
}

int drc_maxpool2d_blocked(const float* x, float* y, int N, int CB, int H, int W, int px, int k, int stride, int OH, int OW, int py,
                          void* stream) {
    if (N < 0 || CB <= 0 || H <= 0 || W <= 0 || k <= 0 || stride <= 0 || OH <= 0 || OW <= 0) return -2;
    if ((OH - 1) * stride >= H || (OW - 1) * stride >= W) return -2;
    const long total = (long)N * CB * OH * OW * 4;
    if (total == 0) return 0;
    if (!x || !y) return -1;
    hipLaunchKernelGGL(maxpool2d_blocked_kernel, dim3(grid_for(total)), dim3(kThreads), 0, (hipStream_t)stream, x, y, N, CB, H, W, px, k, stride, OH, OW, py);
    return done();
}

int drc_copy_blocks(const float* x, float* y, int N, int CB, int64_t vox_per_cb, int y_cb_total, int y_cb_off, void* stream) {
    if (N < 0 || CB <= 0 || vox_per_cb <= 0 || y_cb_off < 0 || y_cb_off + CB > y_cb_total) return -2;
    const long total = (long)N * CB * vox_per_cb * 4;
    if (total == 0) return 0;
    if (!x || !y) return -1;
    hipLaunchKernelGGL(copy_blocks_kernel, dim3(grid_for(total)), dim3(kThreads), 0, (hipStream_t)stream, x, y, N, CB, (long)vox_per_cb, y_cb_total, y_cb_off);
    return done();
}

}
```

disprcnn_amd/engine.py:

```python
import ctypes as C
import functools
import math
from collections import namedtuple

import torch

from . import _lib
from ._lib import DrcTapconvParams

CB = 16
SLACK_FLOATS = 1 << 16
LDS_PER_WAVE_MAX = 38 * 1024
MAX_SLOTS = 112
TIMING = None
SLIDE = {"enabled": True, "max_slots": 112, "ct": 2, "min_od": 3, "min_share": 1, "min_units": 700, "min_units_ct1": 150}


def _stream_ptr(device):
    return C.c_void_p(torch.cuda.current_stream(device).cuda_stream)


def _ptr(t):
    return C.c_void_p(t.data_ptr()) if t is not None else C.c_void_p(0)

# ... 662 lines not shown


def plan_conv2d(x, y, k, stride, pad, dilation, cout, relu):
    assert x.pd == 0 and x.D == 1
    classes, grid = taps_conv((1, k, k), (1, dilation, dilation), (0, pad, pad), (0, x.ph, x.pw)), (1, y.H, y.W)
    R, WT, lds, kname = tapconv_choice(x, classes, stride, grid, cout)
    kernel, ct = KERNELS["tapconv"], None
    tiles = cout_pad_of(cout) // 16
    if k == 3 and DIRECT["enabled"] and DIRECT.get("conv2d", True):
        best = None
        for r in range(1, min(y.H, MAX_SLOTS) + 1):
            for wt in range(1, min(y.W, MAX_SLOTS // r) + 1):
                nvt = -(-(r * wt) // 16)
                ntile = x.N * (-(-y.H // r)) * (-(-y.W // wt))
                waste = (-(-y.H // r)) * (-(-y.W // wt)) * nvt * 16 / (y.H * y.W)
                fill = min(1.0, ntile * tiles / 1024.0) if CONV2D_FILL["enabled"] else 1.0
                key = (round(fill / waste, 2), r * wt, wt)
                if best is None or key > best[0]:
                    best = (key, r, wt)
        R, WT = best[1], best[2]
        nvt = -(-(R * WT) // 16)
        ntile = x.N * (-(-y.H // R)) * (-(-y.W // WT))
        ct = 4 if tiles % 4 == 0 else (2 if tiles % 2 == 0 else 1)
        while ct > 1 and (nvt * ct > 28 or ntile * (tiles // ct) < 700):
            ct //= 2
        kernel, kname = KERNELS["conv2ddirect"], "conv2ddirect_kernel<%d,%d>" % (nvt, ct)
        wtiles = x.N * ((y.H + 1) // 2) * ((y.W + 1) // 2)
        dil_ok = dilation == 1 or (WINO2D["dilated"] and dilation in (2, 4) and y.H % (2 * dilation) == 0 and y.W % (2 * dilation) == 0)
        if (WINO2D["enabled"] and stride == 1 and dil_ok and pad == dilation and (WINO2D["odd"] or not (y.H | y.W) & 1) and
                (x.N * x.n_stride + 2 * x.h_stride) * 4 < 2 ** 32 and wtiles // 64 >= WINO2D["min_chunks"]):
            ct = 2 if tiles % 2 == 0 else 1
            kernel, kname = KERNELS["wino2d"], "wino2d_kernel<%d>" % ct
            if (WINO2D.get("rb") and dilation == 1 and x.cb <= WINO2D["rb_max_cb"] and not (y.H | y.W) & 1 and wtiles // 64 * (cout_pad_of(cout) // 32) >= WINO2D["rb_min_chunks"]
                    and _lib.lib().drc_conv2d_k3_wino_rb_supported(cout_pad_of(cout), y.H, y.W)):
                kernel, ct, kname = KERNELS["wino2d_rb"], None, "wino2d_rb_kernel<%d>" % (7 if y.W == 14 else 14)
    if k == 1 and POINTWISE["enabled"]:
        ntile = -(-(x.N * y.H * y.W) // 16)
        if tiles % 4 == 0 and ntile // 4 * (tiles // 4) >= 2048:
            vc = (4, 4)
        elif tiles % 2 == 0 and ntile // 4 * (tiles // 2) >= 2048:
            vc = (4, 2)
        elif tiles % 2 == 0 and (ntile // 2 * (tiles // 2) >= 1024 or x.cb < 16):
            vc = (2, 2)
        elif ntile // 2 * tiles >= 1024:
            vc = (2, 1)
        else:
            vc = (1, 1)
        kernel, kname = KERNELS["pointwise"], "pointwise_kernel<%d,%d>" % vc
    return ConvPlan(x, y, classes, stride, 1, grid, cout, relu, kernel, kname, (R, WT), lds, ct)


def plan_deconv2d(x, y, k, cout, relu=False):
    assert x.pd == 0 and x.D == 1 and (y.H, y.W) == (2 * x.H, 2 * x.W) and x.ph >= 1 and x.pw >= 1
    classes, grid = taps_deconv2d_s2(k, (0, x.ph, x.pw)), (1, x.H, x.W)
    R, WT, lds, kname = tapconv_choice(x, classes, 1, grid, cout)
    return ConvPlan(x, y, classes, 1, 2, grid, cout, relu, KERNELS["tapconv"], kname, (R, WT), lds)



def cost_volume_blocked(left, right, out, lo4, hi4, in_blocked_pad=0):
    st = _lib.lib().drc_cost_volume_blocked_fwd(_ptr(left), _ptr(right), _ptr(out.storage), out.N, out.C // 2, out.D, out.H, out.W,
                                                lo4, hi4, in_blocked_pad, _stream_ptr(out.device))
    _lib.check(st, "drc_cost_volume_blocked_fwd")


def conv3d_cout1(x, w27, res, out):
    st = _lib.lib().drc_conv3d_cout1_fwd(_ptr(x.storage), _ptr(w27), _ptr(res), _ptr(out), x.N, x.cb, x.D, x.H, x.W,
                                         _stream_ptr(x.device))
    _lib.check(st, "drc_conv3d_cout1_fwd")


TRUNK_S16 = {"enabled": True, "min_tiles": 192, "min_rows": 24}


class BridgedConv2dS16:

    @staticmethod
    def slices(cin):
        if cin in (32, 64, 128):
            return ((0, cin),)
        if cin in (256, 384, 512):
            return tuple((a, a + 128) for a in range(0, cin, 128))
        return None

    @staticmethod
    def worth(N, cin, cout, H, W):
        if not TRUNK_S16["enabled"] or BridgedConv2dS16.slices(cin) is None or cout not in (32, 64, 128, 256, 512) or not S16["enabled"]:
            return False
        if not s16_allowed():
            return False
        tiles = N * -(-H // 28) * -(-W // 28) * (cout // 32)
        return H >= TRUNK_S16["min_rows"] and tiles >= TRUNK_S16["min_tiles"]

    def __init__(self, N, cin, cout, H, W, relu, device, cache):
        self.bounds = self.slices(cin)
        if self.bounds is None or not s16_supported(self.bounds[0][1] - self.bounds[0][0], cout, 1, H, W, "2d"):
            raise ValueError("BridgedConv2dS16: unsupported shape")
        self.N, self.cin, self.cout, self.H, self.W, self.device = N, cin, cout, H, W, device

        def shared(tag, ch):
            k = (tag, N, ch, H, W)
            if k not in cache:
                cache[k] = RS16(N, ch, 1, H, W, 0, device)
            return cache[k]
        self.x16 = [shared(("x", i), b - a) for i, (a, b) in enumerate(self.bounds)]
        self.y16 = [shared(("y", i), cout) for i in range(min(2, len(self.bounds)))]
        last = len(self.bounds) - 1
        self.plans = [ConvPlanS16(N, b - a, cout, 1, H, W, bool(relu) and i == last, device=device, kind="2d") for i, (a, b) in enumerate(self.bounds)]

    def run(self, x, packs, shift, zero_shift, y):
        if (x.C, x.H, x.W, y.C, y.H, y.W) != (self.cin, self.H, self.W, self.cout, self.H, self.W) or x.N < self.N or y.N < self.N:
            raise ValueError("BridgedConv2dS16.run: tensors differ from the plan")
        prev = None
        for i, ((a, b), pl, (w16, sc16)) in enumerate(zip(self.bounds, self.plans, packs)):
            self.x16[i].from_blocked(x if len(self.bounds) == 1 else BlockedSlice(x, a // CB, b - a))
            out = self.y16[i & 1]
            pl.run(self.x16[i], w16, sc16, shift if i == 0 else zero_shift, y16=out, res=prev)
            prev = out
        prev.to_blocked(y)


def head_gather(S, scale, res, out):
    N, D, H, W = out.shape
    st = _lib.lib().drc_head_gather_fwd(_ptr(S), _ptr(res), _ptr(out), N, D, H, W, C.c_float(scale), _stream_ptr(out.device))
    _lib.check(st, "drc_head_gather_fwd")


def head_gather_rows(rows, scales, res, out):
    N, D, H, W = out.shape
    if not 1 <= len(rows) <= 3 or len(scales) != len(rows):
        raise ValueError("head_gather_rows: 1 to 3 heads, one scale each")
    for r in rows:
        if r.dtype != torch.float32 or r.numel() < N * D * H * W * 4 or not r.is_contiguous():
            raise ValueError("head_gather_rows: rows = contiguous fp32 buffers of N*D*H*W*4")
    if out.dtype != torch.float32 or not out.is_contiguous() or (res is not None and (res.dtype != torch.float32 or res.shape != out.shape or not res.is_contiguous())):
        raise ValueError("head_gather_rows: out / res = contiguous fp32 [N,D,H,W]")
    ptrs = [_ptr(r) for r in rows] + [None] * (3 - len(rows))
    sc = [C.c_float(float(s)) for s in scales] + [C.c_float(0.0)] * (3 - len(rows))
    st = _lib.lib().drc_head_gather_rows_fwd(ptrs[0], ptrs[1], ptrs[2], sc[0], sc[1], sc[2], len(rows), _ptr(res), _ptr(out), N, D, H, W, _stream_ptr(out.device))
    _lib.check(st, "drc_head_gather_rows_fwd")


def head_gather_planar(planes, scales, res, out):
    N, D, H, W = out.shape
    if not 1 <= len(planes) <= 3 or len(scales) != len(planes):
        raise ValueError("head_gather_planar: 1 to 3 heads, one scale each")
    for r in planes:
        if r.dtype != torch.float32 or r.numel() < N * D * H * W * 9 or not r.is_contiguous():
            raise ValueError("head_gather_planar: planes = contiguous fp32 buffers of N*D*9*H*W")
    if out.dtype != torch.float32 or not out.is_contiguous() or (res is not None and (res.dtype != torch.float32 or res.shape != out.shape or not res.is_contiguous())):
        raise ValueError("head_gather_planar: out / res = contiguous fp32 [N,D,H,W]")
    ptrs = [_ptr(r) for r in planes] + [None] * (3 - len(planes))
    sc = [C.c_float(float(s)) for s in scales] + [C.c_float(0.0)] * (3 - len(planes))
    st = _lib.lib().drc_head_gather_planar_fwd(ptrs[0], ptrs[1], ptrs[2], sc[0], sc[1], sc[2], len(planes), _ptr(res), _ptr(out), N, D, H, W, _stream_ptr(out.device))
    _lib.check(st, "drc_head_gather_planar_fwd")


def upsample_softargmin(cost, disp, maxdisp, mindisp):
    N, Dp, Hp, Wp = cost.shape
    _, H, W = disp.shape
    st = _lib.lib().drc_upsample_softargmin_fwd(_ptr(cost), _ptr(disp), N, Dp, Hp, Wp, maxdisp - mindisp, H, W, mindisp,
                                                _stream_ptr(cost.device))
    _lib.check(st, "drc_upsample_softargmin_fwd")


def _geom8(t):
    import ctypes
    base = getattr(t, "base", None)
    return (ctypes.c_int * 10)(t.N, t.cb, t.D, t.H, t.W, t.pd, t.ph, t.pw, base.cb if base is not None else t.cb,
                                t.cb_off if base is not None else 0)


_BN_SCRATCH = {}
BN_MAX_CHUNKS = 512


def bn_scratch(dev, cb):
    key = (dev, torch.cuda.current_stream(dev).cuda_stream if dev.type == "cuda" else 0, cb)
    buf = _BN_SCRATCH.get(key)
    if buf is None:
        buf = _BN_SCRATCH[key] = torch.zeros(BN_MAX_CHUNKS * cb * 32 + cb * 32 * 33, dtype=torch.float32, device=dev)
    return buf


_WGRAD_SCRATCH = {}


def wgrad_scratch(dev):
    key = (dev, torch.cuda.current_stream(dev).cuda_stream if dev.type == "cuda" else 0)
    buf = _WGRAD_SCRATCH.get(key)
    if buf is None:
        buf = _WGRAD_SCRATCH[key] = torch.empty(_lib.WGRAD_SCRATCH_FLOATS, dtype=torch.float32, device=dev)
    return buf


_SCRATCH = {}


def scratch(dev, tag, floats):
    key = (dev, torch.cuda.current_stream(dev).cuda_stream if dev.type == "cuda" else 0, tag)
    buf = _SCRATCH.get(key)
    if buf is None or buf.numel() < floats:
        buf = _SCRATCH[key] = torch.empty(int(floats), dtype=torch.float32, device=dev)
    return buf


def bn_batch_stats(raw):
    dev = raw.device
    C16 = raw.cb * CB
    M = raw.N * raw.D * raw.H * raw.W
    stats = torch.empty(2, C16, dtype=torch.float32, device=dev)
    st = _lib.lib().drc_bn_stats_blocked(_ptr(raw.storage), _geom8(raw), _ptr(stats), _ptr(bn_scratch(dev, raw.cb)), _stream_ptr(dev))
    _lib.check(st, "drc_bn_stats_blocked")
    return stats[0], stats[1] / M, M


def bn_batch_stats_raw(raw):
    dev = raw.device
    stats = torch.empty(2, raw.cb * CB, dtype=torch.float32, device=dev)
    st = _lib.lib().drc_bn_stats_blocked(_ptr(raw.storage), _geom8(raw), _ptr(stats), _ptr(bn_scratch(dev, raw.cb)), _stream_ptr(dev))
    _lib.check(st, "drc_bn_stats_blocked")
    return stats, raw.N * raw.D * raw.H * raw.W


def bn_finalize(stats, count, bn, cout):
    dev = stats.device
    invstd = torch.empty(stats.shape[1], dtype=torch.float32, device=dev)
    track = bn.track_running_stats and bn.running_mean is not None
    st = _lib.lib().drc_bn_finalize(_ptr(stats), stats.shape[1], cout, count, float(bn.eps), float(bn.momentum),
                                    _ptr(bn.running_mean) if track else None, _ptr(bn.running_var) if track else None,
                                    _ptr(bn.num_batches_tracked) if track else None, _ptr(invstd), _stream_ptr(dev))
    _lib.check(st, "drc_bn_finalize")
    if track:
        for t in (bn.running_mean, bn.running_var, bn.num_batches_tracked):
            torch.autograd.graph.increment_version(t)
    return invstd


def bn_apply(raw, y, res, mean, invstd, gamma, beta, relu):
    st = _lib.lib().drc_bn_apply_blocked(_ptr(raw.storage), _geom8(raw), _ptr(y.storage), _geom8(y),
                                         _ptr(res.storage) if res is not None else None, _geom8(res) if res is not None else None,
                                         _ptr(mean), _ptr(invstd), _ptr(gamma), _ptr(beta), int(relu), _stream_ptr(raw.device))
    _lib.check(st, "drc_bn_apply_blocked")


CB16 = 32


class Blocked16:

    def __init__(self, N, C_, D, H, W, pd, ph, pw, device, storage=None):
        self.N, self.C, self.D, self.H, self.W = N, C_, D, H, W
        self.pd, self.ph, self.pw = pd, ph, pw
        self.cb = (C_ + CB16 - 1) // CB16
        self.Dp, self.Hp, self.Wp = D + 2 * pd, H + 2 * ph, W + 2 * pw
        self.h_stride = self.Wp * CB16
        self.d_stride = self.Hp * self.h_stride
        self.cb_stride = self.Dp * self.d_stride
        self.n_stride = self.cb * self.cb_stride
        self.numel = N * self.n_stride
        if storage is None:
            self.storage = torch.zeros(self.numel + 2 * SLACK_FLOATS, dtype=torch.float16, device=device)
        else:
            if storage.numel() < self.numel + 2 * SLACK_FLOATS:
                raise ValueError("Blocked16: the given storage is too small for this geometry")
            self.storage = storage.narrow(0, 0, self.numel + 2 * SLACK_FLOATS)
        self.device = device

    @property
    def interior_off(self):
        return self.pd * self.d_stride + self.ph * self.h_stride + self.pw * CB16

    def view6(self):
        return self.storage[: self.numel].view(self.N, self.cb, self.Dp, self.Hp, self.Wp, CB16)

    def from_dense(self, dense):
        v = self.view6()
        n, c = dense.shape[:2]
        pad_c = self.cb * CB16 - c
        d = torch.nn.functional.pad(dense.to(torch.float16), (0, 0, 0, 0, 0, 0, 0, pad_c)) if pad_c else dense.to(torch.float16)
        d = d.view(n, self.cb, CB16, self.D, self.H, self.W).permute(0, 1, 3, 4, 5, 2)
        v[:, :, self.pd:self.pd + self.D, self.ph:self.ph + self.H, self.pw:self.pw + self.W, :] = d
        return self

    def to_dense(self):
        v = self.view6()[:, :, self.pd:self.pd + self.D, self.ph:self.ph + self.H, self.pw:self.pw + self.W, :]
        return v.permute(0, 1, 5, 2, 3, 4).reshape(self.N, self.cb * CB16, self.D, self.H, self.W)[:, : self.C].float()


class Blocked16Slice:

    def __init__(self, base, cb_off, C_):
        self.base, self.cb_off = base, cb_off
        self.N, self.C, self.D, self.H, self.W = base.N, C_, base.D, base.H, base.W
        self.pd, self.ph, self.pw = base.pd, base.ph, base.pw
        self.cb = (C_ + CB16 - 1) // CB16
        assert cb_off >= 0 and cb_off + self.cb <= base.cb
        self.Dp, self.Hp, self.Wp = base.Dp, base.Hp, base.Wp
        self.h_stride, self.d_stride, self.cb_stride, self.n_stride = base.h_stride, base.d_stride, base.cb_stride, base.n_stride
        self.storage = base.storage[cb_off * base.cb_stride:]
        self.interior_off = base.interior_off
        self.device = base.device


def dense_to_blocked16(dense, out):
    require_gpu(dense, "dense_to_blocked16")
    dense = dense.contiguous().float()
    st = _lib.lib().drc_dense_to_blocked16(_ptr(dense), _ptr(out.storage), out.N, out.C, out.H, out.W, out.ph, out.pw, _stream_ptr(out.device))
    _lib.check(st, "drc_dense_to_blocked16")
    return out


def plan_conv2d16(x, y, k, stride, pad, dilation, cout, relu):
    assert x.pd == 0 and x.D == 1
    return ConvPlan16(x, y, taps_conv((1, k, k), (1, dilation, dilation), (0, pad, pad), (0, x.ph, x.pw)), stride, 1, (1, y.H, y.W), cout, relu)

# ... 467 lines not shown
```

disprcnn_amd/modeling/psmnet/runtime.py:

```python
import functools
import operator
import weakref
from collections import OrderedDict

import torch

from ... import engine as E
from .schedule import CONCAT, REGRESSOR_HEADS, REGRESSOR_SITES, REGRESSOR_TENSORS, STRIDE, concat_slots, trunk_sites
from .submodule import SPP_BRANCHES, TRUNK_STAGES

TRUNK = trunk_sites()
_HEAD_OF = {h.site.plan: h for h in REGRESSOR_HEADS}
_LAYER_KINDS = tuple(dict.fromkeys((s.kind, s.cin, s.cout, s.level) for s in REGRESSOR_SITES))

GRAPH_MAX_UNITS = 96
GRAPH_MAX_ENTRIES = 16
GRAPH_CAPTURE_AFTER = 2
MAX_SLOTS = 4
WS_MAX_PLANS = 48


_UNIT_AFFINE = {}
_TENSOR_VERSION = operator.attrgetter("_version")
_TENSOR_PTR = torch.Tensor.data_ptr
# ... 101 lines not shown

    @staticmethod
    def inputs(rt, ws, N, full):
        pool = ws["pool"]
        ws["t"].lazy["cost"] = lambda: pool.blocked("cost", N, 64, *full, 1, 1, 1)

    @staticmethod
    def alloc(pool, name, N, c, dims):
        return pool.blocked(name, N, c, *dims, 1, 1, 1)

    @staticmethod
    def head_tensors(ws, N, full):
        pass

    @staticmethod
    def plan(rt, ws, s, N, dims):
        t = ws["t"]
        x = E.Blocked.geometry(N, s.cin, *dims, 1, 1, 1, rt.device) if s.costvol else t[s.x]
        ws["p"][s.plan] = (E.plan_deconv3d(x, t[s.y], s.cout, s.relu) if s.kind == "up" else
                           E.plan_conv3d(x, t[s.y], STRIDE[s.kind], s.cout, s.relu))

    @staticmethod
    def entry(ws, s):
        return (s.plan, s.wname, s.x, s.y, s.res)

    @staticmethod
    def runner(rt, ws, W):
        return functools.partial(rt._site, ws, W)

    @staticmethod
    def first(ws, W, run, cv):
        if cv is not None:
            c, pl = W["dres0.0"], ws["p"]["dres0.0"]
            pl.run_costvol(cv[0], cv[1], cv[2], c.w16_for(pl), c.scale, c.shift, ws["t"]["d0a"])
        else:
            run(*ws["first"])

    @staticmethod
    def heads(rt, ws, W, run):
        t, prev = ws["t"], None
        for e, h in ws["heads"]:
            run(*e)
            E.conv3d_cout1(t[h.cls_t], W[h.weight], prev, t[h.costk])
            prev = t[h.costk]
        return t["costk1"], t["costk2"], t["costk3"]


class _Blocked16(_Blocked32):
    tag, costk_last = "3d16", False

    @staticmethod
    def inputs(rt, ws, N, full):
        if E.COSTVOL16_FUSED["enabled"]:
            ws["t"]["pair"] = ws["pool"].blocked16("pair", N, 64, 1, *full[1:], 1, 1, 1)
        else:
            ws["t"]["cost"] = ws["pool"].blocked16("cost", N, 64, *full, 1, 1, 1)

    @staticmethod
    def alloc(pool, name, N, c, dims):
        return pool.blocked16(name, N, c, *dims, 1, 1, 1)

    @staticmethod
    def plan(rt, ws, s, N, dims):
        t, p = ws["t"], ws["p"]
        if s.costvol and "pair" in t:
            p[s.plan] = E.plan_conv3d16_costvol(t["pair"], t[s.y], 0, s.cout, s.relu)
        elif s.kind == "up":
            p[s.plan] = E.plan_deconv3d16(t[s.x], t[s.y], s.cout, s.relu)
        else:
            p[s.plan] = E.plan_conv3d16(t[s.x], t[s.y], STRIDE[s.kind], s.cout, s.relu)
        if s.plan in _HEAD_OF:
            p[_HEAD_OF[s.plan].weight] = E.plan_conv3d16_cout1(t[s.y])

    @staticmethod
    def entry(ws, s):
        t = ws["t"]
        return (ws["p"][s.plan], s.wname, t["pair" if s.costvol and "pair" in t else s.x], t[s.y], t[s.res] if s.res else None)

    @staticmethod
    def runner(rt, ws, W):
        W16 = rt._weights16(W)

        def run(pl, wname, x, y, res):
            c = W[wname]
            pl.run(x, W16[wname], c.scale, c.shift, y, res)
        return run

    @staticmethod
    def first(ws, W, run, cv):
        run(*ws["first"])

    @staticmethod
    def heads(rt, ws, W, run):
        t, p, W16, prev = ws["t"], ws["p"], rt._weights16(W), None
        for e, h in ws["heads"]:
            run(*e)
            p[h.weight].run(t[h.cls_t], W16[h.weight], None, None, t[h.costk], prev)
            prev = t[h.costk]
        return t["costk1"], t["costk2"], t["costk3"]


class _SplitF16(_Blocked32):
    tag, costk_last = "3ds16", False

    @staticmethod
    def inputs(rt, ws, N, full):
        for name in ("featL", "featR"):
            ws["t"][name] = ws["pool"].rs16(name, N, 32, 1, *full[1:], 0)

    @staticmethod
    def alloc(pool, name, N, c, dims):
        return None if name.startswith("cls_t") else pool.rs16(name, N, c, *dims, 1)

    @staticmethod
    def head_tensors(ws, N, full):
        t, pool = ws["t"], ws["pool"]
        ws["fused_heads"] = E.HEAD_FUSED["enabled"] and full[2] % 28 == 0 and full[0] >= 6 and full[0] % 3 == 0
        if ws["fused_heads"]:
            t["hs"] = pool.dense("hs", N, *full, 27 if full[2] == 28 else 12)
        else:
            for h in REGRESSOR_HEADS:
                t[h.cls_t] = pool.blocked(h.cls_t, N, 32, *full, 1, 1, 1)

    @staticmethod
    def plan(rt, ws, s, N, dims):
        ws["p"][s.plan] = E.ConvPlanS16(N, s.cin, s.cout, *dims, s.relu, cv=s.costvol, device=rt.device, kind=s.kind)

    @staticmethod
    def entry(ws, s):
        t = ws["t"]
        return (ws["p"][s.plan], s.wname, None if s.costvol else t[s.x], None if s.plan in _HEAD_OF else t[s.y], t[s.res] if s.res else None)

    @staticmethod
    def runner(rt, ws, W):
        def run(pl, wname, x, y16, res, **kw):
            c = W[wname]
            w16, sc16 = c.s16()
            pl.run(x, w16, sc16, c.shift, y16=y16, res=res, **kw)
        return run

    @staticmethod
    def first(ws, W, run, cv):
        run(*ws["first"], left=ws["t"]["featL"], right=ws["t"]["featR"], lo4=cv)

    @staticmethod
    def heads(rt, ws, W, run):
        t, prev = ws["t"], None
        h16 = rt._head_weights_s16() if ws["fused_heads"] else None
        if h16 is not None and E.HEAD_ROWS["enabled"] and t["costk3"].shape[-1] == 28:
            rows = t["hs"].view(3, -1)
            planar = bool(ws["heads"][0][0][0].head_flat())
            for e, h in ws["heads"]:
                run(*e, head=(h16[h.k][0], rows[h.k - 1]), head_layout=E.HEAD_PLANAR if planar else E.HEAD_ROWS_LAYOUT)
            (E.head_gather_planar if planar else E.head_gather_rows)([rows[0], rows[1], rows[2]], [h16[k][1] for k in (1, 2, 3)], None, t["costk3"])
            return None, None, t["costk3"]
        for e, h in ws["heads"]:
            if h16 is not None:
                run(*e, head=(h16[h.k][0], t["hs"]))
                E.head_gather(t["hs"], h16[h.k][1], prev, t[h.costk])
            else:
                run(*e, y32=t[h.cls_t])
                E.conv3d_cout1(t[h.cls_t], W[h.weight], prev, t[h.costk])
            prev = t[h.costk]
        return t["costk1"], t["costk2"], t["costk3"]


class PSMNetRuntime:
    def __init__(self, model, device):
        self.model = model
        self.device = device
        self._weights_version = None
        self._folds_version = None
        self._w = None
        self._ws = OrderedDict()
        self._pools = {}
        self._training = False
        self._tape = None
        self._held = {}
        self._slot = 0
        self._graphs = OrderedDict()
        self._graph_seen = {}
        self._epoch = 0
        self._guard = None
        self._s16_used = False

    def _pick_slot(self):
        for s in range(MAX_SLOTS):
            if s not in self._held:
                return s
        raise RuntimeError(f"PSMNet: {MAX_SLOTS} train-mode forward passes are waiting for their backward; run backward() (or drop "
                           f"their outputs) first, or raise disprcnn_amd.modeling.psmnet.runtime.MAX_SLOTS")

    def _slotted(self, key):
        return key if self._slot == 0 else key + (("slot", self._slot),)

    def _hold(self, slot):
        class _Token:
            pass
        tok = _Token()
        self._held[slot] = id(tok)
        weakref.finalize(tok, PSMNetRuntime._release, weakref.ref(self), slot, id(tok))
        return tok

    @staticmethod
    def _release(rt_ref, slot, tok_id):
        rt = rt_ref() if isinstance(rt_ref, weakref.ref) else rt_ref
        if rt is not None and rt._held.get(slot) == tok_id:
            del rt._held[slot]

    def invalidate(self):
        self._weights_version = None

    def _pool_for(self, gkey, n):
        pool = self._pools.get(gkey)
        if pool is None or pool.cap < n:
            if pool is not None:
                for k in [k for k, w in self._ws.items() if w.get("pool") is pool]:
                    del self._ws[k]
            pool = self._pools[gkey] = E.WorkspacePool(E.bucket_units(n), self.device)
            self._epoch += 1
        return pool

    def _ws_get(self, key):
        ws = self._ws.get(key)
        if ws is not None:
            self._ws.move_to_end(key)
        return ws

    def _ws_put(self, key, ws):
        self._ws[key] = ws
        while len(self._ws) > WS_MAX_PLANS:
            self._ws.popitem(last=False)
        return ws

    def workspace_bytes(self):
        return sum(p.nbytes() for p in self._pools.values())

    @staticmethod
    def _stamp(*wss):
        for ws in wss:
            ws["pool"].gen += 1

    @staticmethod
    def _generations(*wss):
        return [(ws["pool"], ws["pool"].gen) for ws in wss]

    @staticmethod
    def _check_generations(gens):
        for pool, gen in gens:
            if pool.gen != gen:
                raise RuntimeError(
                    "PSMNet backward: the workspace of this forward pass was reused by a later forward (another batch of the "
                    "same geometry, or an eval pass) before backward() ran, so the saved activations are gone (retain_graph / a "
                    "second backward through the same forward is not supported: run the forward again).")

    def _slots(self, kind):
        cache = self.__dict__.setdefault("_slot_cache", {})
        sl = cache.get(kind)
        if sl is not None and all(d.get(n) is t for d, n, t in sl):
            return sl
        sl = []
        for mod in self.model.modules():
            d = mod._parameters if kind == "p" else mod._buffers
            sl.extend((d, n, t) for n, t in d.items() if t is not None)
        cache[kind] = sl
        return sl

    def _tensors(self, kind):
        sl = self._slots(kind)
        cache = self.__dict__["_slot_cache"]
        ent = cache.get("t" + kind)
        if ent is None or ent[0] is not sl:
            ent = cache["t" + kind] = (sl, [t for _, _, t in sl])
        return ent[1]

    def _version(self):
        ts = self._tensors("p")
        return (list(map(_TENSOR_VERSION, ts)), list(map(_TENSOR_PTR, ts)))

    def _buffers_version(self):
        ts = self._tensors("b")
        return (list(map(_TENSOR_VERSION, ts)), list(map(_TENSOR_PTR, ts)))

    def _compile(self):
        v = self._version()
        if self._w is not None and v == self._weights_version:
            if not self._training:
                vb = self._buffers_version()
                if vb != self._folds_version:
                    for c in self._w.values():
                        if isinstance(c, _Conv):
                            c.refold()
                    self._folds_version = vb
                    self._epoch += 1
            return self._w
        m, dev = self.model, self.device
        W = {}

        def cb3(name, seq, transposed=False):
            W[name] = _Conv(seq[0], seq[1], dev, transposed)

        for s in REGRESSOR_SITES:
            cb3(s.wname, m.get_submodule(s.prefix), s.kind == "up")
        for h in REGRESSOR_HEADS:
            W[h.weight] = E.pack_weight_cout1(m.get_submodule(h.weight).weight.detach().to(device=dev, dtype=torch.float32))
        fe = m.feature_extraction
        for s in TRUNK.stem + TRUNK.blocks:
            cb3(s.wname, fe.get_submodule(s.prefix))
        for name, _ in SPP_BRANCHES:
            cb3(f"fe.{name}", getattr(fe, name)[1])
        cb3("fe.lastconv.0", fe.lastconv[0])
        W["fe.lastconv.2"] = _Conv(fe.lastconv[2], None, dev)
        self._w, self._weights_version, self._folds_version = W, v, None
        self._epoch += 1
        if not self._training:
            for c in W.values():
                if isinstance(c, _Conv):
# ... 18 lines not shown
            ws["raw"][plan] = raw
        pl.run(t[x], c.w, c.unit_scale, c.zero_shift, raw, None, relu=False, w16=c.w16_for(pl))
        bn = c.bn
        fused = (bn.momentum is not None and bn.running_mean is not None and bn.running_mean.device == raw.device and
                 bn.running_mean.dtype == torch.float32 and bn.running_mean.is_contiguous() and bn.running_var.is_contiguous())
        if fused:
            stats, M = E.bn_batch_stats_raw(raw)
            mean = stats[0]
            invstd = E.bn_finalize(stats, M, bn, c.cout)
        else:
            mean, var, M = E.bn_batch_stats(raw)
            invstd = torch.rsqrt(var + bn.eps)
            with torch.no_grad():
                bn.num_batches_tracked += 1
                mom = bn.momentum if bn.momentum is not None else 1.0 / float(bn.num_batches_tracked)
                unb = var[: c.cout] * (M / max(M - 1, 1))
                bn.running_mean.mul_(1 - mom).add_(mean[: c.cout].to(bn.running_mean.device), alpha=mom)
                bn.running_var.mul_(1 - mom).add_(unb.to(bn.running_var.device), alpha=mom)
        relu = bool(pl.p.relu)
        E.bn_apply(raw, yt, rs, mean, invstd, c.gamma, c.beta, relu)
        ws.setdefault("saved", {})[plan] = (mean, invstd, M)
        if self._tape is not None:
            self._tape.append(("site", ws, plan, wname, x, y, res))

    def _ws3d(self, ad, N, Dp, Hp, Wp):
        key = self._slotted((ad.tag, N, Dp, Hp, Wp))
        ws = self._ws_get(key)
        if ws is not None:
            return ws
        pool = self._pool_for(self._slotted((ad.tag, Dp, Hp, Wp)), N)
        full = (Dp, Hp, Wp)
        half = tuple(-(-s // 2) for s in full)
        quart = tuple(-(-s // 2) for s in half)
        if tuple(2 * s for s in half) != full or tuple(2 * s for s in quart) != half:
            raise ValueError(f"cost-volume dims {full} must be divisible by 4 (D,H,W multiples of 16; SURVEY 8)")
        dims = (full, half, quart)
        t, p = _LazyTensors(), {}
        ws = dict(t=t, p=p, pool=pool, ad=ad)
        pending = iter(REGRESSOR_HEADS)

        def costk(h):
            t[h.costk] = pool.dense(h.costk, N, *full)

        ad.inputs(self, ws, N, full)
        for name, c, lvl in REGRESSOR_TENSORS:
            v = ad.alloc(pool, name, N, c, dims[lvl])
            if v is not None:
                t[name] = v
            if not ad.costk_last and name.endswith(".c4"):
                costk(next(pending))
        for h in pending:
            costk(h)
        ad.head_tensors(ws, N, full)
        for s in REGRESSOR_SITES:
            ad.plan(self, ws, s, N, dims[s.level])
        body = [ad.entry(ws, s) for s in REGRESSOR_SITES if s.plan not in _HEAD_OF]
        ws.update(first=body[0], body=body[1:], heads=[(ad.entry(ws, h.site), h) for h in REGRESSOR_HEADS])
        ws["flops"] = sum(pl.flops for pl in p.values()) + (0 if REGRESSOR_HEADS[0].weight in p else 3 * 2 * 27 * 32 * N * Dp * Hp * Wp)
        return self._ws_put(key, ws)

    def _fuse_costvol(self, ws, training):
        return bool(not training and self._tape is None and E.WINO["fuse_costvol"] and ws["p"]["dres0.0"].wino)

    def _regress(self, ws, W, cv=None):
        ad = ws["ad"]
        run = ad.runner(self, ws, W)
        ad.first(ws, W, run, cv)
        for e in ws["body"]:
            run(*e)
        return ad.heads(self, ws, W, run)

    @staticmethod
    def _s16_layers(Dp, Hp, Wp):
        dims = ((Dp, Hp, Wp), (Dp // 2, Hp // 2, Wp // 2), (Dp // 4, Hp // 4, Wp // 4))
        return [(kind, cin, cout, dims[level]) for kind, cin, cout, level in _LAYER_KINDS]

    def _use_s16(self, training, Dp, Hp, Wp):
        mode = getattr(self.model, "regressor_math", "auto")
        if mode not in ("auto", "f32", "f16x2"):
            raise ValueError("PSMNet.regressor_math must be 'auto', 'f32' or 'f16x2'")
        ok = (not training and self._tape is None and Dp % 4 == 0 and Hp % 4 == 0 and Wp % 4 == 0 and Wp > 14 and
              all(E.s16_supported(ci, co, *dims, kind=kind) for kind, ci, co, dims in self._s16_layers(Dp, Hp, Wp)))
        if mode == "f16x2" and not ok:
            raise RuntimeError("PSMNet.regressor_math = 'f16x2': eval only; volume dims D', H', W' multiples of 4, W' >= 16 (the cost-volume layer runs on 28-wide tiles)")
        return self._s16_choice(ok and mode != "f32", mode, "regressor_math")

    def _s16_choice(self, use, mode, what):
        if use and not E.s16_allowed():
            if mode == "f16x2":
                raise RuntimeError(f"PSMNet.{what} = 'f16x2': a value left the split-f16 range (|v| > 65504) in an enclosing guarded pass")
            return False
        if use:
            self._s16_used = True
        return use

    def _head_weights_s16(self):
        if getattr(self, "_h16_version", None) == self._weights_version and getattr(self, "_h16", None) is not None:
            return self._h16
        from ... import s16 as S
        out = {}
        for k in (1, 2, 3):
            wp, wexp = S.pack_head_weight_s16(getattr(self.model, f"classif{k}")[2].weight)
            out[k] = (wp.to(self.device), 2.0 ** -wexp)
        self._h16, self._h16_version = out, self._weights_version
        return out

    def _weights16(self, W):
        if getattr(self, "_w16_version", None) == self._weights_version and getattr(self, "_w16", None) is not None:
            return self._w16
        m, dev = self.model, self.device
        out = {}
        for name, c in W.items():
            if isinstance(c, _Conv):
                out[name] = E.pack_weight16(c.conv.weight.detach().to(device=dev, dtype=torch.float32), c.transposed)
        for k in (1, 2, 3):
            out[f"classif{k}.2"] = E.pack_weight16(getattr(m, f"classif{k}")[2].weight.detach().to(device=dev, dtype=torch.float32))
        self._w16, self._w16_version = out, self._weights_version
        return out

    def _costvol16(self, ws, mn, mx, left=None, right=None, in_pad=-1, feat16=None, right_first=0):
        t = ws["t"]
        dst, lo, hi = (t["pair"], 0, 1) if "pair" in t else (t["cost"], mn // 4, mx // 4)
        if "pair" in t:
            ws["p"]["dres0.0"].costvol_lo4 = mn // 4
        if feat16 is not None:
            E.cost_volume16_from16(feat16, right_first, dst, lo, hi)
        else:
            E.cost_volume16_blocked(left, right, dst, lo, hi, in_pad)

    def _use_f16(self, training):
        mode = getattr(self.model, "regressor_storage", "f32")
        if mode not in ("f32", "f16"):
            raise ValueError("PSMNet.regressor_storage must be 'f32' or 'f16'")
        if mode == "f16" and training:
            raise RuntimeError("the fp16-storage regressor is an inference path (BASELINE configs[3]); train in fp32 like the reference")
        return mode == "f16"

    def _features_f16(self):
        mode = getattr(self.model, "feature_storage", "f32")
        if mode not in ("f32", "f16"):
            raise ValueError("PSMNet.feature_storage must be 'f32' or 'f16'")
        return mode == "f16"

    def _check_disp(self):
        mx, mn = self.model.maxdisp, self.model.mindisp
        if (mx - mn) % 16 != 0 or mx % 4 != 0 or mn % 4 != 0:
            raise ValueError("maxdisp/mindisp must be multiples of 4 with a range divisible by 16 (SURVEY 8, a1)")
        return mx, mn

    def _heads(self, costs, N, H, W, mx, mn, training):
        outs = []
        for c in (costs if training else costs[2:]):
            d = torch.empty(N, H, W, dtype=torch.float32, device=self.device)
            E.upsample_softargmin(c, d, mx, mn)
            outs.append(d)
        return tuple(outs) if training else outs[0]

    def _graph_mode(self, n_units, training):
        mode = getattr(self.model, "graph_eval", "auto")
        if mode not in ("auto", True, False):
            raise ValueError("PSMNet.graph_eval must be 'auto', True or False")
        if training or mode is False or self._held or torch.is_grad_enabled() or n_units == 0 or E.TIMING is not None:
            return False
        if torch.cuda.is_current_stream_capturing():
            return False
        return mode is True or n_units <= GRAPH_MAX_UNITS

    def _replay(self, key, inputs, fn):
        from ...utils.graph import GraphedStep
        n = inputs[0].shape[0]
        nb = E.bucket_units(n)
        key = (nb,) + tuple(key)
        ent = self._graphs.get(key)
        if ent is not None and ent["epoch"] == self._epoch:
            out = self._replay_launch(ent, inputs, n)
            self._compile()
            if ent["epoch"] == self._epoch:
                self._graphs.move_to_end(key)
                return out
            ent = self._graphs.get(key)
        else:
            self._compile()
        if ent is not None and ent["epoch"] != self._epoch:
            del self._graphs[key]
            ent = None
        if ent is None:
            seen = self._graph_seen.get(key, 0) + 1
            if len(self._graph_seen) > 256:
                self._graph_seen.clear()
            self._graph_seen[key] = seen
            if seen < GRAPH_CAPTURE_AFTER:
                return fn(*inputs)
            static = [torch.zeros((nb,) + tuple(t.shape[1:]), dtype=t.dtype, device=t.device) for t in inputs]
            for s_, t in zip(static, inputs):
                s_[:n].copy_(t)
            self._s16_used = False
            fn(*static)
            step = GraphedStep(lambda: fn(*static), warmup=1)
            ent = dict(epoch=self._epoch, static=static, step=step, filled=n, s16=self._s16_used, guard=E.guard_in_scope())
            self._graphs[key] = ent
            self._graph_seen.pop(key, None)
            while len(self._graphs) > GRAPH_MAX_ENTRIES:
                self._graphs.popitem(last=False)
        else:
            self._graphs.move_to_end(key)
        return self._replay_launch(ent, inputs, n)

    def _replay_launch(self, ent, inputs, n):
        for s_, t in zip(ent["static"], inputs):
            s_[:n].copy_(t)
            if ent["filled"] > n:
                s_[n:ent["filled"]].zero_()
        ent["filled"] = n
        if ent["s16"]:
            self._s16_used = True
            g = E.guard_in_scope()
            if g is not None:
                g.used = True
        return ent["step"]()[:n].clone()

    def _guarded(self, training, fn):
        if training or self.device.type != "cuda":
            return fn()
        if self._guard is None:
            self._guard = E.OverflowGuard(self.device)
        m = self.model
        strict = "f16x2" in (getattr(m, "regressor_math", "auto"), getattr(m, "feature_math", "auto"))
        return E.guarded(self._guard, fn, strict=strict, what="PSMNet (split-f16 regressor / feature CNN)",
                         enabled=bool(getattr(m, "overflow_check", True)))

    def _graph_key_tail(self):
        m = self.model
        return (m.maxdisp, m.mindisp, getattr(m, "regressor_math", "auto"), getattr(m, "regressor_storage", "f32"),
                getattr(m, "feature_storage", "f32"), getattr(m, "feature_math", "auto"),
                E.S16["enabled"], E.HEAD_FUSED["enabled"], E.LASTCONV_S16["enabled"], E.TRUNK_S16["enabled"], E.CV_WIDE["enabled"], E.HEAD_ROWS["enabled"], tuple(sorted(E.HEAD_FLAT.items())), E.s16_allowed(),
                id(E.guard_in_scope()))

    def forward_features(self, fl, fr, out_hw, training=False):
        return self._guarded(training, lambda: self._forward_features_once(fl, fr, out_hw, training))

    def forward_images(self, left, right, training=False):
        return self._guarded(training, lambda: self._forward_images_once(left, right, training))

    def _forward_features_once(self, fl, fr, out_hw, training=False):
        self._training = bool(training)
        self._slot = self._pick_slot()
        if fl.is_cuda and fl.shape == fr.shape and fl.dim() == 4 and self._graph_mode(fl.shape[0], training):
            key = ("feat", tuple(fl.shape[1:]), tuple(out_hw)) + self._graph_key_tail()
            return self._replay(key, (fl, fr), lambda a, b: self._forward_features_impl(a, b, out_hw, False))
        if training and torch.is_grad_enabled():
            params = [p for _, _, p in self._slots("p") if p.requires_grad and not self._is_fe_param(p)]
            if fl.requires_grad or fr.requires_grad or params:
                return _RegressorTrainFn.apply(self, tuple(out_hw), fl, fr, *params)
        return self._forward_features_impl(fl, fr, out_hw, training)

    def _is_fe_param(self, p):
        ids = getattr(self, "_fe_ids", None)
        if ids is None:
            ids = self._fe_ids = {id(q) for q in self.model.feature_extraction.parameters()}
        return id(p) in ids

    def _forward_features_impl(self, fl, fr, out_hw, training):
        E.require_gpu(fl, "PSMNet features"); E.require_gpu(fr, "PSMNet features")
        mx, mn = self._check_disp()
        N, C, Hp, Wp = fl.shape
        H, W = out_hw
        if C != 32:
            raise ValueError("feature maps must have 32 channels")
        if N == 0:
            z = torch.empty(0, H, W, dtype=torch.float32, device=self.device)
            return (z, z.clone(), z.clone()) if training else z
        if not self._use_f16(training) and self._use_s16(training, (mx - mn) // 4, Hp, Wp):
            ws = self._ws3d(_SplitF16, N, (mx - mn) // 4, Hp, Wp)
            self._stamp(ws)
            ws["t"]["featL"].from_dense(fl)
            ws["t"]["featR"].from_dense(fr)
            Wt = self._compile()
            return self._heads(self._regress(ws, Wt, mn // 4), N, H, W, mx, mn, False)
        Wt = self._compile()
        if self._use_f16(training):
            ws = self._ws3d(_Blocked16, N, (mx - mn) // 4, Hp, Wp)
            self._stamp(ws)
            self._costvol16(ws, mn, mx, fl.contiguous(), fr.contiguous())
            return self._heads(self._regress(ws, Wt), N, H, W, mx, mn, False)
        ws = self._ws3d(_Blocked32, N, (mx - mn) // 4, Hp, Wp)
        self._stamp(ws)
        cv = None
        if self._fuse_costvol(ws, training):
            pool = ws["pool"]
            cv = (pool.blocked("featL", N, 32, 1, Hp, Wp, 0, 1, 1).from_dense(fl),
                  pool.blocked("featR", N, 32, 1, Hp, Wp, 0, 1, 1).from_dense(fr), mn // 4)
        else:
            E.cost_volume_blocked(fl.contiguous(), fr.contiguous(), ws["t"]["cost"], mn // 4, mx // 4, 0)
        costs = self._regress(ws, Wt, cv)
        self._last_train = (ws, Wt, costs, mx, mn, (H, W))
        self._last_gens = self._generations(ws)
        return self._heads(costs, N, H, W, mx, mn, training)

    def _ws2d(self, N, H, W, side=None, f16=False):
        tag = "2d16" if f16 else "2d"
        key = self._slotted((tag, N, H, W) if side is None else (tag, N, H, W, side))
        ws = self._ws_get(key)
        if ws is not None:
            return ws
        if H % 4 or W % 4 or H // 4 < 56 or W // 4 < 56:
            raise ValueError("PSMNet needs H,W multiples of 4 and >= 224 (fixed AvgPool2d(56), reference submodule.py:76)")
        pool = self._pool_for(self._slotted((tag, H, W) if f16 else (tag, H, W, side)), N)
        names = iter(range(1 << 30))
        if f16:
            B2 = lambda c, h, w, pad=1: pool.blocked16(("t16", next(names)), N, c, 1, h, w, 0, pad, pad)
            plan, Slice, cb = E.plan_conv2d16, E.Blocked16Slice, 32
        else:
            B2 = lambda c, h, w, pad=1: pool.blocked(("t", next(names)), N, c, 1, h, w, 0, pad, pad)
            plan, Slice, cb = E.plan_conv2d, E.BlockedSlice, 16
        hw = ((H, W), (H // 2, W // 2), (H // 4, W // 4))
        parts = {TRUNK.raw: CONCAT[0], TRUNK.skip: CONCAT[1]}
        t, p = {}, {}
        t["img"] = B2(3, H, W)
        for s in TRUNK.stem:
            t[s.y] = B2(s.cout, *hw[s.level])
        for s in TRUNK.stem:
            p[s.wname] = plan(t[s.x], t[s.y], s.k, s.stride, s.pad, s.dilation, s.cout, s.relu)
        t["cat"] = B2(320, *hw[2])
        sched = []
        for s in TRUNK.blocks:
            if s.y in parts:
                _, off, ch = parts[s.y]
                t[s.y] = Slice(t["cat"], off // cb, ch)
            else:
                t[s.y] = B2(s.cout, *hw[s.level], s.halo)
            p[s.wname] = plan(t[s.x], t[s.y], s.k, s.stride, s.pad, s.dilation, s.cout, s.relu)
            sched.append((s.wname, s.wname, s.x, s.y, s.res))
        return self._ws_put(key, self._ws2d_tail(t, p, B2, plan, cb, pool, sched, TRUNK.skip, *hw[2]))

    @staticmethod
    def _ws2d_tail(t, p, B2, plan, cb, pool, sched, skip, H4, W4):
        slot = concat_slots(cb)
        spp = []
        for name, k in SPP_BRANCHES:
            oh, ow = H4 // k, W4 // k
            t[name + ".pool"] = B2(128, oh, ow, 0)
            t[name + ".conv"] = B2(32, oh, ow, 0)
            p["fe." + name] = plan(t[name + ".pool"], t[name + ".conv"], 1, 1, 0, 1, 32, True)
            spp.append((name, k, oh, ow, slot[name]))
        t["last0"] = B2(128, H4, W4, 0)
        t["feat"] = B2(32, H4, W4, 1)
        p["fe.lastconv.0"] = plan(t["cat"], t["last0"], 3, 1, 1, 1, 128, True)
        p["fe.lastconv.2"] = plan(t["last0"], t["feat"], 1, 1, 0, 1, 32, False)
        return dict(t=t, p=p, pool=pool, sched=sched, spp=spp, skip=skip, dims=(H4, W4),
                    flops=sum(pl.flops for pl in p.values()) + sum(e[1].flops for e in sched if e[0] == "s16"))

    def _use_s16_2d(self, training, H, W):
        mode = getattr(self.model, "feature_math", "auto")
        if mode not in ("auto", "f32", "f16x2"):
            raise ValueError("PSMNet.feature_math must be 'auto', 'f32' or 'f16x2'")
        ok = (not training and self._tape is None and H % 4 == 0 and W % 4 == 0 and H // 4 >= 56 and W // 4 >= 56 and
              E.s16_supported(32, 32, 1, H // 2, W // 2, "2d") and E.s16_supported(64, 64, 1, H // 4, W // 4, "2d") and
              E.s16_supported(64, 128, 1, H // 4, W // 4, "2d") and E.s16_supported(128, 128, 1, H // 4, W // 4, "2d"))
        if mode == "f16x2" and not ok:
            raise RuntimeError("PSMNet.feature_math = 'f16x2': eval only; H, W multiples of 4 and >= 224 (the reference's AvgPool2d(56), submodule.py:76)")
        return self._s16_choice(ok and mode != "f32", mode, "feature_math")

    def _ws2d_eval(self, N, H, W):
        return self._ws2d_s16(N, H, W) if self._use_s16_2d(False, H, W) else self._ws2d(N, H, W)

    def _ws2d_s16(self, N, H, W):
        key = self._slotted(("2ds16", N, H, W))
        ws = self._ws_get(key)
        if ws is not None:
            return ws
        pool = self._pool_for(self._slotted(("2ds16", H, W)), N)
        names = iter(range(1 << 30))
        B2 = lambda c, h, w, pad=1: pool.blocked(("t", next(names)), N, c, 1, h, w, 0, pad, pad)
        S2 = lambda name, c, h, w: pool.rs16(("s", name), N, c, 1, h, w, 0)
        H2, W2, H4, W4 = H // 2, W // 2, H // 4, W // 4
        t, p = {}, {}
        t["img"] = B2(3, H, W)
        t["f0"] = B2(32, H2, W2)
        p["fe.firstconv.0"] = E.plan_conv2d(t["img"], t["f0"], 3, 2, 1, 1, 32, True)
        t["cat"] = B2(320, H4, W4)
        sched = []
        plans = {}

        def s16(cin, cout, h, w, wname, x, y, res, relu):
            k = (cin, cout, h, w, relu)
            if k not in plans:
                plans[k] = E.ConvPlanS16(N, cin, cout, 1, h, w, relu, device=self.device, kind="2d")
            sched.append(("s16", plans[k], wname, x, y, res))
# ... 322 lines not shown
```

include/disprcnn_hip.h:

```cpp
#ifndef DISPRCNN_HIP_H
#define DISPRCNN_HIP_H

#include <stdint.h>

#ifdef __cplusplus
extern "C" {
#endif

#define DRC_MAX_CLASSES 8
#define DRC_CB 16

const char* drc_version(void);

int drc_cost_volume_fwd(const float* left, const float* right, float* cost,
                        int N, int C, int Dp, int Hp, int Wp, int lo4, int hi4, void* stream);

int drc_cost_volume_bwd(const float* gcost, float* gleft, float* gright,
                        int N, int C, int Dp, int Hp, int Wp, int lo4, int hi4, void* stream);

int drc_cost_volume_blocked_fwd(const float* left, const float* right, float* cost_blk,
                                int N, int C, int Dp, int Hp, int Wp, int lo4, int hi4,
                                int in_blocked_pad, void* stream);

int drc_dense_to_blocked(const float* dense, float* blk, int N, int C, int D, int H, int W,
                         int pd, int ph, int pw, void* stream);
int drc_blocked_to_dense(const float* blk, float* dense, int N, int C, int D, int H, int W,
                         int pd, int ph, int pw, void* stream);

typedef struct drc_tap_class {
    int32_t nd, nh, nw;
    int32_t dd0, dh0, dw0;
    int32_t sd, sh, sw;
    int32_t wbase, wsd, wsh, wsw;
    int32_t out_off_d, out_off_h, out_off_w;
} drc_tap_class;

typedef struct drc_tapconv_params {
    const float* x;
    const float* w;
    const float* scale;
    const float* shift;
    const float* res;
    float* y;
    int64_t x_n_stride, x_cb_stride, x_d_stride, x_h_stride;
    int64_t y_n_stride, y_cb_stride, y_d_stride, y_h_stride;
    int64_t y_off0;
    int64_t r_n_stride, r_cb_stride, r_d_stride, r_h_stride;
    int64_t r_off0;
    int32_t N, OD, OH, OW;
    int32_t in_mul, out_mul;
    int32_t cb_in;
    int32_t cout_pad;
    int32_t R, WT;
    int32_t relu;
    int32_t n_classes;
    int32_t lds_bytes_per_wave;
    int32_t reserved;
    drc_tap_class cls[DRC_MAX_CLASSES];
} drc_tapconv_params;

int drc_tapconv_fwd(const drc_tapconv_params* p, void* stream);

int drc_tapconv3d_direct_fwd(const drc_tapconv_params* p, int cout_tiles_per_wave, void* stream);

int drc_deconv3d_k3s2_fwd(const drc_tapconv_params* p, void* stream);

int drc_conv3d_k3s2_direct_fwd(const drc_tapconv_params* p, int cout_tiles_per_wave, void* stream);

int drc_deconv3d_k3s2_direct_fwd(const drc_tapconv_params* p, int cout_tiles_per_wave, void* stream);
int drc_deconv3d_k3s2_direct_s16_fwd(const drc_tapconv_params* p, void* y16, uint32_t* ovf, void* stream);

int drc_conv3d_k3_wino_fwd(const drc_tapconv_params* p, int cout_tiles_per_wave, void* stream);

int drc_conv3d_k3_wino_rb_supported(int cout_pad, int OD, int OH, int OW);
int drc_conv3d_k3_wino_rb_fwd(const drc_tapconv_params* p, void* stream);
int drc_pack_weights_wino_rb(const float* w, int cout, int cin, int transposed, int flip, float* out, void* stream);
int drc_conv2d_k3_wino_rb_supported(int cout_pad, int OH, int OW);
int drc_conv2d_k3_wino_rb_fwd(const drc_tapconv_params* p, void* stream);
int drc_pack_weights_wino2d_rb(const float* w, int cout, int cin, int transposed, int flip, float* out, void* stream);

typedef struct drc_costvol_src {
    const float* left;
    const float* right;
    int64_t n_stride, cb_stride, h_stride;
    int32_t cbi;
    int32_t pad;
    int32_t lo4;
    int32_t Wp;
} drc_costvol_src;

int drc_conv3d_k3_wino_costvol_fwd(const drc_tapconv_params* p, const drc_costvol_src* cv, int cout_tiles_per_wave, void* stream);
int drc_conv3d_k3_wino_rb_costvol_fwd(const drc_tapconv_params* p, const drc_costvol_src* cv, void* stream);

int drc_conv2d_k3_wino_fwd(const drc_tapconv_params* p, int cout_tiles_per_wave, void* stream);
int drc_pack_weights_wino2d(const float* w, int cout, int cin, int transposed, int flip, float* out, void* stream);

int drc_pack_weights_wino(const float* w, int cout, int cin, int transposed, int flip, float* out, void* stream);

int drc_conv2d_k3_direct_fwd(const drc_tapconv_params* p, int cout_tiles_per_wave, void* stream);
int drc_conv2d_k3s2_stem_fwd(const float* x, int N, int H, int W, const float* w_packed, int cout_pad, const float* scale, const float* shift,
                             float* y, int64_t y_n_stride, int64_t y_cb_stride, int64_t y_h_stride, int64_t y_off0, int OH, int OW, int relu,
                             void* stream);

int drc_conv2d_k1_fwd(const drc_tapconv_params* p, void* stream);

int drc_conv3d_cout1_fwd(const float* x, const float* w, const float* res, float* out,
                         int N, int cb_in, int D, int H, int W, void* stream);

int drc_upsample_softargmin_fwd(const float* cost, float* disp, int N, int Dp, int Hp, int Wp,
                                int D, int H, int W, int mindisp, void* stream);
int drc_upsample_softargmin_form(int Dp, int Hp, int Wp, int D, int H, int W);

int drc_pack_weights(const float* w, int cout, int cin, int K, int transposed, int flip, float* out_tap, float* out_t16, void* stream);

int drc_avgpool2d_blocked(const float* x, float* y, int N, int CB, int H, int W, int px,
                          int k, int OH, int OW, int py, void* stream);
int drc_avgpool2d_blocked_slice(const float* x, float* y, int N, int CB, int H, int W, int px, int k, int OH, int OW, int py,
                                int x_cb_total, int x_cb_off, void* stream);
int drc_bilinear_up_blocked(const float* x, float* y, int N, int CB, int IH, int IW, int px,
                            int OH, int OW, int py, int y_cb_total, int y_cb_off, void* stream);
int drc_bilinear_resize_blocked(const float* x, float* y, int N, int CB, int IH, int IW, int px, int OH, int OW, int py,
                                int y_cb_total, int y_cb_off, int align_corners, void* stream);
int drc_maxpool2d_blocked(const float* x, float* y, int N, int CB, int H, int W, int px, int k, int stride, int OH, int OW, int py,
                          void* stream);
int drc_copy_blocks(const float* x, float* y, int N, int CB, int64_t vox_per_cb,
                    int y_cb_total, int y_cb_off, void* stream);

int drc_roi_align_fwd(const float* input, const float* rois, float* out, int K, int C, int H, int W, int PH, int PW,
                      float spatial_scale, int sampling_ratio, const float* mean, const float* stdv, void* stream);
#define DRC_FPN_MAX_LEVELS 8
typedef struct {
    const float* feat[DRC_FPN_MAX_LEVELS];
    int32_t H[DRC_FPN_MAX_LEVELS], W[DRC_FPN_MAX_LEVELS];
    float scale[DRC_FPN_MAX_LEVELS];
    int32_t n_levels;
} drc_fpn_pyramid;
int drc_roi_align_fpn_fwd(const drc_fpn_pyramid* pyr, const float* rois, const int32_t* levels, float* out, int K, int C, int PH, int PW,
                          int sampling_ratio, void* stream);
int drc_roi_align_bwd(const float* grad_out, const float* rois, float* grad_in, int K, int C, int H, int W, int PH, int PW,
                      float spatial_scale, int sampling_ratio, void* stream);
int drc_roi_align_fpn_bwd(const drc_fpn_pyramid* grad_pyr, const float* grad_out, const float* rois, const int32_t* levels, int K, int C, int PH,
                          int PW, int sampling_ratio, void* stream);

int drc_align_roi_pairs(const float* left_boxes, const float* right_boxes, const int32_t* img_idx, int R, int img_w, int img_h,
                        float* rois_left, float* rois_right, int32_t* geom, void* stream);

int drc_conv16_fwd(const drc_tapconv_params* p, void* stream);
int drc_conv16_k3_tile_supported(const drc_tapconv_params* p);
int drc_dense_to_blocked16(const float* x, void* y16, int N, int C, int H, int W, int ph, int pw, void* stream);
int drc_avgpool2d_blocked16_slice(const void* x16, void* y16, int N, int CB32, int H, int W, int px, int k, int OH, int OW, int py,
                                  int x_cb_total, int x_cb_off, void* stream);
int drc_bilinear_up_blocked16(const void* x16, void* y16, int N, int CB32, int IH, int IW, int px, int OH, int OW, int py, int y_cb_total,
                              int y_cb_off, void* stream);
int drc_cost_volume16_from16(const void* feat16, void* cost16, int N, int right_first_unit, int C, int Dp, int Hp, int Wp, int mindisp4,
                             int maxdisp4, int feat_pad, void* stream);
int drc_conv16_k3_tile_fwd(const drc_tapconv_params* p, void* stream);

int drc_conv16_k3_costvol_fwd(const drc_tapconv_params* p, int mindisp4, void* stream);

typedef struct drc_s16conv_params {
    const void* x;
    const void* w;
    const float* scale;
    const float* shift;
    const void* res;
    void* y16;
    float* y32;
    const void* left;
    const void* right;
    int32_t N, D, H, W;
    int32_t cin, cout, relu;
    int32_t lo4;
    int32_t dil;
    float* head;
    const void* w1;
    uint32_t* ovf;
    int32_t head_rows;
} drc_s16conv_params;
#define DRC_HEAD_SLOTS 0
#define DRC_HEAD_ROWS 1
#define DRC_HEAD_PLANAR 2
int drc_conv3d_k3_s16_supported(int cin, int cout, int D, int H, int W);
int drc_conv3d_k3_s16_fwd(const drc_s16conv_params* p, void* stream);
int drc_conv3d_k3_s16_wide(const drc_s16conv_params* p);
int drc_conv3d_k3_s16_flat(const drc_s16conv_params* p);
int drc_conv3d_k3_s16_wide_fwd(const drc_s16conv_params* p, void* stream);
int drc_head_gather_fwd(const float* S, const float* res, float* cost, int N, int D, int H, int W, float scale, void* stream);
int drc_head_gather_rows_fwd(const float* rows0, const float* rows1, const float* rows2, float scale0, float scale1, float scale2, int nheads,
                             const float* res, float* cost, int N, int D, int H, int W, void* stream);
int drc_head_gather_planar_fwd(const float* s0, const float* s1, const float* s2, float scale0, float scale1, float scale2, int nheads,
                               const float* res, float* cost, int N, int D, int H, int W, void* stream);
int drc_conv3d_k3s2_s16_supported(int cin, int cout, int D, int H, int W);
int drc_conv3d_k3s2_s16_fwd(const drc_s16conv_params* p, void* stream);
int drc_deconv3d_k3s2_s16_supported(int cin, int cout, int D, int H, int W);
int drc_deconv3d_k3s2_s16_fwd(const drc_s16conv_params* p, void* stream);
int drc_conv2d_k3_s16_supported(int cin, int cout, int H, int W, int dil);
int drc_conv2d_k3_s16_fwd(const drc_s16conv_params* p, void* stream);
int drc_rs16_from_dense(const float* x, void* y16, int N, int C, int D, int H, int W, int pd, uint32_t* ovf, void* stream);
int drc_rs16_from_blocked(const float* xb, void* y16, int N, int C, int D, int H, int W, int pd_in, int ph_in, int pw_in, int cb16_total,
                          int cb16_off, int pd, uint32_t* ovf, void* stream);
int drc_rs16_to_dense(const void* y16, float* x, int N, int C, int D, int H, int W, int pd, void* stream);
int drc_rs16_to_blocked(const void* y16, float* xb, int N, int C, int D, int H, int W, int pd_out, int ph_out, int pw_out, int cb16_total,
                        int cb16_off, int pd, void* stream);
int drc_conv16_k3s2_tile_supported(const drc_tapconv_params* p);
int drc_conv16_k3s2_tile_fwd(const drc_tapconv_params* p, void* stream);
int drc_deconv16_k3s2_tile_supported(const drc_tapconv_params* p);
int drc_deconv16_k3s2_tile_fwd(const drc_tapconv_params* p, void* stream);
int drc_cost_volume16_blocked_fwd(const float* left, const float* right, void* cost16, int N, int C, int Dp, int Hp, int Wp,
                                  int mindisp4, int maxdisp4, int in_blocked_pad, void* stream);

int drc_nms_sorted_fwd(const float* boxes_sorted, int n, float thresh, int strict, uint64_t* mask_ws, uint8_t* keep, void* stream);
int drc_nms_sorted_batch_fwd(const float* boxes_sorted, int sets, int n, float thresh, int strict, uint64_t* mask_ws, uint8_t* keep, void* stream);
int drc_nms_sorted_pair_joint_fwd(const float* boxes_sorted, int n, float thresh, int strict, int max_keep, uint64_t* mask_ws,
                                  uint8_t* keep_joint, void* stream);

int drc_box_decode_fwd(const float* codes, const float* boxes, float* out, int64_t rows, int groups, int per_group, const float* weights4,
                       float xform_clip, float img_w, float img_h, void* stream);
int drc_srpn_proposals_fwd(const float* logits, const float* regression, const float* anchors, const float* image_wh, int N, int A, int H,
                           int W, int64_t total_anchors, int64_t level_offset, float xform_clip, float* scores, float* left, float* right,
                           void* stream);

int drc_roi_train_targets_fwd(const float* disp_maps, const uint8_t* gt_masks, const float* mask_probs, int mask_size, int padding,
                              float mask_thresh, const float* det_boxes, const float* rois_left, const int32_t* geom, int R, int H, int W,
                              int res, float* targets, uint8_t* masks, void* stream);

int drc_disparity_paste_fwd(const float* disp, int S, const int32_t* boxes, const int32_t* roi_offsets, int B, int H, int W, int flags,
                            const float* mask, float* out, void* stream);
int drc_roi_depth_maps_fwd(const float* disp, int S, const int32_t* boxes, const float* fuxb, int R, int H, int W, float* out, void* stream);

int drc_disparity_resize_fwd(const float* src, int IH, int IW, float* dst, int OH, int OW, int mode, void* stream);

int64_t drc_linear_packed_floats(int R, int K);
int drc_linear_pack_rows(const float* a, int R, int K, float* out, void* stream);
int64_t drc_linear_scratch_floats(int M, int N, int K);
int drc_linear_fwd(const float* x, const float* w, const float* bias, float* y, int M, int N, int K, int relu, float* scratch,
                   int64_t scratch_floats, void* stream);
int drc_linear_pack_cols(const float* a, int R, int K, float* out, void* stream);
int drc_relu_dropout_fwd(const float* x, const float* draws, float* y, int64_t total, float p, int relu, void* stream);
int64_t drc_act_bwd_rows_scratch_doubles(int M, int N);
int drc_act_bwd_rows(const float* dy, const float* y, const float* draws, float p, int relu, int M, int N, int fold, float* dz, float* db,
                     double* scratch, int64_t scratch_doubles, void* stream);
int64_t drc_act_bwd_blocked_scratch_doubles(int units, int C, int H);
int drc_act_bwd_blocked(const float* dy, const float* y, int relu, int units, int C, int H, int W, int ph, int pw, float* dz, float* db,
                        double* scratch, int64_t scratch_doubles, void* stream);

#define DRC_LOSS_SCRATCH_FLOATS ((size_t)1024 * 8)
int drc_psm_loss_sums(const float* pred1, const float* pred2, const float* pred3, const float* target, const uint8_t* mask,
                      int64_t numel, float* sums5, float* scratch, void* stream);
int drc_psm_loss_grad(const float* pred, const float* target, const uint8_t* mask, int64_t numel, const float* sums5, float weight,
                      const float* grad_scale, float* grad_pred, void* stream);

#define DRC_BN_MAX_CHUNKS 512
#define DRC_BN_SCRATCH_FLOATS(CB) ((size_t)DRC_BN_MAX_CHUNKS * (CB) * 32 + (size_t)(CB) * 32 * 33)
int drc_bn_stats_blocked(const float* x, const int* geom8, float* stats, float* scratch, void* stream);
int drc_bn_finalize(const float* stats, int C16, int C, long long count, float eps, float momentum, float* running_mean, float* running_var,
                    long long* num_batches_tracked, float* invstd, void* stream);
int drc_bn_apply_blocked(const float* x, const int* geom_x, float* y, const int* geom_y, const float* res, const int* geom_r,
                         const float* mean, const float* invstd, const float* gamma, const float* beta, int relu, void* stream);

int64_t drc_upsample_softargmin_bwd_scratch_floats(int N, int Dp, int Hp, int Wp, int H, int W);
int drc_upsample_softargmin_bwd(const float* cost, const float* grad_disp, float* grad_cost, int N, int Dp, int Hp, int Wp, int D, int H,
                                int W, int mindisp, float* scratch, int64_t scratch_floats, void* stream);
int drc_conv3d_cout1_bwd_data(const float* grad_out, const float* w, float* grad_x_blk, int N, int cb_in, int D, int H, int W,
                              int accumulate, void* stream);
#define DRC_COUT1_WGRAD_SCRATCH_FLOATS(cb_in) ((size_t)1024 * (cb_in) * 27 * 16)
int drc_conv3d_cout1_bwd_weight(const float* x_blk, const float* grad_out, float* grad_w, int N, int cb_in, int D, int H, int W,
                                float* scratch, void* stream);
int drc_bn_bwd_reduce(const float* dy, const int* geom_dy, const float* y, const int* geom_y, const float* raw, const int* geom_raw,
                      const float* mean, const float* invstd, int relu, float* sums, float* scratch , void* stream);
int drc_bn_bwd_apply(const float* dy, const int* geom_dy, const float* y, const int* geom_y, const float* raw, const int* geom_raw,
                     const float* mean, const float* invstd, const float* gamma, const float* sums, float inv_count, int relu, float* draw,
                     const int* geom_draw, float* dres, const int* geom_dres, int dres_accumulate, void* stream);

#define DRC_WGRAD_SCRATCH_FLOATS ((size_t)(1024 + 3 * 64) * 49 * 256)
typedef struct drc_wgrad_params {
    const float* a;
    const float* b;
    float* gw;
    int64_t a_n_stride, a_cb_stride, a_d_stride, a_h_stride;
    int64_t b_n_stride, b_cb_stride, b_d_stride, b_h_stride, b_off0;
    int32_t N, OD, OH, OW;
    int32_t in_mul, cb_a, cb_b;
    int32_t nd, nh, nw, dd0, dh0, dw0, sd, sh, sw;
    int32_t R, WT, lds_bytes_per_wave;
    int32_t overwrite;
    float* scratch;
    int64_t scratch_floats;
} drc_wgrad_params;
int drc_tapconv_wgrad(const drc_wgrad_params* p, void* stream);

int drc_bilinear_up_blocked_bwd(const float* grad_y, const int* geom_y, float* grad_x, const int* geom_x, void* stream);
int drc_avgpool2d_blocked_bwd(const float* grad_y, const int* geom_y, float* grad_x, const int* geom_x, int k, void* stream);

#define DRC_SRPN_MAX_LEVELS 8
typedef struct drc_srpn_levels {
    int32_t n_levels, N, A, C;
    int32_t cap, reserved;
    int32_t H[DRC_SRPN_MAX_LEVELS], W[DRC_SRPN_MAX_LEVELS];
    int64_t pix_off[DRC_SRPN_MAX_LEVELS + 1];
    const float* left[DRC_SRPN_MAX_LEVELS];
    const float* right[DRC_SRPN_MAX_LEVELS];
    const float* hidden[DRC_SRPN_MAX_LEVELS];
    int64_t hidden_n_stride[DRC_SRPN_MAX_LEVELS];
    const float* glogits[DRC_SRPN_MAX_LEVELS];
    const float* gbbox[DRC_SRPN_MAX_LEVELS];
} drc_srpn_levels;
int drc_srpn_active_pixels(const drc_srpn_levels* lv, const uint8_t* pos, const uint8_t* neg, int32_t* row_pix, int32_t* counts,
                           int32_t* index, void* stream);
int drc_srpn_gather_rows(const drc_srpn_levels* lv, const int32_t* row_pix, const float* g_obj, const float* g_box, float* T, float* Xcol,
                         float* G, void* stream);
int drc_srpn_col2im(const drc_srpn_levels* lv, const float* dxcol, const int32_t* index, int view_mask, void* stream);

#ifdef __cplusplus
}
#endif
#endif
```

Baseline: 66170 ROI cost-volumes/s.

## Fuse planar head gather with upsample and soft-argmin into one banded kernel

```diff
diff --git a/disprcnn_amd/_lib.py b/disprcnn_amd/_lib.py
--- a/disprcnn_amd/_lib.py
+++ b/disprcnn_amd/_lib.py
@@ -128,6 +128,7 @@
     "drc_conv3d_cout1_fwd": (_I, [_P, _P, _P, _P, _I, _I, _I, _I, _I, _P]),
     "drc_upsample_softargmin_fwd": (_I, [_P, _P, _I, _I, _I, _I, _I, _I, _I, _I, _P]),
     "drc_upsample_softargmin_form": (_I, [_I, _I, _I, _I, _I, _I]),
+    "drc_upsample_softargmin_fwd_sel": (_I, [_P, _P, _I, _I, _I, _I, _I, _I, _I, _I, _I, _P]),
     "drc_avgpool2d_blocked": (_I, [_P, _P, _I, _I, _I, _I, _I, _I, _I, _I, _I, _P]),
     "drc_pack_weights": (_I, [_P, _I, _I, _I, _I, _I, _P, _P, _P]),
     "drc_avgpool2d_blocked_slice": (_I, [_P, _P, _I, _I, _I, _I, _I, _I, _I, _I, _I, _I, _I, _P]),
@@ -169,6 +170,9 @@
     "drc_head_gather_fwd": (_I, [_P, _P, _P, _I, _I, _I, _I, C.c_float, _P]),
     "drc_head_gather_rows_fwd": (_I, [_P, _P, _P, C.c_float, C.c_float, C.c_float, _I, _P, _P, _I, _I, _I, _I, _P]),
     "drc_head_gather_planar_fwd": (_I, [_P, _P, _P, C.c_float, C.c_float, C.c_float, _I, _P, _P, _I, _I, _I, _I, _P]),
+    "drc_disp_tail_planar_form": (_I, [_I, _I, _I, _I, _I, _I, _I]),
+    "drc_disp_tail_planar_fwd": (_I, [_P, _P, _P, C.c_float, C.c_float, C.c_float, _I, _P, _P, _P, _I, _I, _I, _I, _I, _I, _I, _I, _P]),
+    "drc_disp_tail_planar_rows": (_I, [_I, _I, C.POINTER(C.c_int)]),
     "drc_conv2d_k3_s16_supported": (_I, [_I, _I, _I, _I, _I]),
     "drc_conv2d_k3_s16_fwd": (_I, [C.POINTER(DrcS16ConvParams), _P]),
     "drc_deconv3d_k3s2_direct_s16_fwd": (_I, [C.POINTER(DrcTapconvParams), _P, _P, _P]),
diff --git a/disprcnn_amd/csrc/build.py b/disprcnn_amd/csrc/build.py
--- a/disprcnn_amd/csrc/build.py
+++ b/disprcnn_amd/csrc/build.py
@@ -3,7 +3,7 @@
 import sys
 
 HERE = os.path.dirname(os.path.abspath(__file__))
-SOURCES = ["tapconv.hip", "tapdirect.hip", "wino3d.hip", "wino3d_rb.hip", "wino2d.hip", "tapdeconv.hip", "deconvdirect.hip", "downdirect.hip", "stemconv.hip", "pointwise.hip", "linear.hip", "head_train.hip", "srpn_train.hip", "volume_ops.hip", "cout1_mfma.hip", "roi_ops.hip", "nms_ops.hip", "det_ops.hip", "post_ops.hip", "train_ops.hip", "bwd_ops.hip", "wgrad.hip", "wgrad_slide.hip", "conv16.hip", "conv16t.hip", "conv16x.hip", "ops16.hip", "convs16.hip", "convs16w.hip", "convs16d.hip", "convs16u.hip", "convs16r.hip", "s16_ops.hip"]
+SOURCES = ["tapconv.hip", "tapdirect.hip", "wino3d.hip", "wino3d_rb.hip", "wino2d.hip", "tapdeconv.hip", "deconvdirect.hip", "downdirect.hip", "stemconv.hip", "pointwise.hip", "linear.hip", "head_train.hip", "srpn_train.hip", "volume_ops.hip", "cout1_mfma.hip", "roi_ops.hip", "nms_ops.hip", "det_ops.hip", "post_ops.hip", "train_ops.hip", "bwd_ops.hip", "wgrad.hip", "wgrad_slide.hip", "conv16.hip", "conv16t.hip", "conv16x.hip", "ops16.hip", "convs16.hip", "convs16w.hip", "convs16d.hip", "convs16u.hip", "convs16r.hip", "s16_ops.hip", "disp_tail.hip"]
 LIB = os.path.join(HERE, "libdisprcnn_hip.so")
 HIPCC = os.environ.get("HIPCC", "/opt/rocm/bin/hipcc")
 FLAGS = ["--offload-arch=gfx950", "-O3", "-std=c++17", "-fPIC", "-ffp-contract=off", "-Wall", "-Wno-unused-function", "-Wno-pass-failed"]
diff --git a/disprcnn_amd/csrc/disp_tail.h b/disprcnn_amd/csrc/disp_tail.h
--- /dev/null
+++ b/disprcnn_amd/csrc/disp_tail.h
@@ -0,0 +1,113 @@
+#pragma once
+#include <hip/hip_runtime.h>
+
+namespace {
+
+struct HeadRows {
+    const float* rows[3];
+    float scale[3];
+};
+
+template <int NH>
+static __device__ __forceinline__ float head_planar_voxel(const HeadRows& hr, float c, long plane, int y, int x, int H, int W) {
+    const long HW = (long)H * W;
+    const int e = y * W + x;
+    const bool xm = x > 0, xp = x + 1 < W, ym = y > 0, yp = y + 1 < H;
+    const int dm = xm ? -1 : 0, dp = xp ? 1 : 0, du = ym ? -W : 0, dd = yp ? W : 0;
+    float v[NH][9];
+#pragma unroll
+    for (int k = 0; k < NH; ++k) {
+        const float* p = hr.rows[k] + plane * 9 * HW + e;
+#pragma unroll
+        for (int j = 0; j < 9; ++j) v[k][j] = p[j * HW + (j < 3 ? du : j < 6 ? 0 : dd) + (j % 3 == 0 ? dm : j % 3 == 2 ? dp : 0)];
+    }
+#pragma unroll
+    for (int k = 0; k < NH; ++k) {
+        const float* q = v[k];
+        const float l0 = xm ? q[0] : 0.f, l3 = xm ? q[3] : 0.f, l6 = xm ? q[6] : 0.f;
+        const float r2 = xp ? q[2] : 0.f, r5 = xp ? q[5] : 0.f, r8 = xp ? q[8] : 0.f;
+        const float t0 = (l0 + q[1]) + r2;
+        const float t1a = l3 + q[4];
+        const float t1b = r5;
+        const float t2 = (l6 + q[7]) + r8;
+        float s = (ym ? t0 : 0.f) + (t1a + t1b);
+        if (yp) s += t2;
+        c = hr.scale[k] * s + c;
+    }
+    return c;
+}
+
+typedef float f32x2 __attribute__((ext_vector_type(2)));
+template <int P> struct SaLanes;
+template <> struct SaLanes<1> {
+    typedef float type;
+    static __device__ __forceinline__ float pack(const float* s) { return s[0]; }
+    static __device__ __forceinline__ float lane(float v, int) { return v; }
+};
+template <> struct SaLanes<2> {
+    typedef f32x2 type;
+    static __device__ __forceinline__ f32x2 pack(const float* s) { f32x2 r; r.x = s[0]; r.y = s[1]; return r; }
+    static __device__ __forceinline__ float lane(f32x2 v, int j) { return j ? v.y : v.x; }
+};
+static __device__ __forceinline__ float sa_max(float a, float b) { return fmaxf(a, b); }
+static __device__ __forceinline__ f32x2 sa_max(f32x2 a, f32x2 b) { f32x2 r; r.x = fmaxf(a.x, b.x); r.y = fmaxf(a.y, b.y); return r; }
+static __device__ __forceinline__ float sa_exp2(float a) { return __builtin_amdgcn_exp2f(a); }
+static __device__ __forceinline__ f32x2 sa_exp2(f32x2 a) { f32x2 r; r.x = __builtin_amdgcn_exp2f(a.x); r.y = __builtin_amdgcn_exp2f(a.y); return r; }
+static __device__ __forceinline__ float sa_fma(float a, float b, float c) { return fmaf(a, b, c); }
+static __device__ __forceinline__ f32x2 sa_fma(f32x2 a, f32x2 b, f32x2 c) { return __builtin_elementwise_fma(a, b, c); }
+
+template <int DP, int D, int P>
+static __device__ __forceinline__ void softargmin_columns(const float* rows, int cy0, int Hp, int Wp, int W, float sy, float sx, const int* pix,
+                                                          int mindisp, float* out) {
+    typedef SaLanes<P> L;
+    typedef typename L::type V;
+    int o00[P], o01[P], o10[P], o11[P];
+    float txs[P], tys[P];
+#pragma unroll
+    for (int j = 0; j < P; ++j) {
+        const int y = pix[j] / W, x = pix[j] - y * W;
+        const float fy = sy * y, fx = sx * x;
+        const int y0 = (int)fy, x0 = (int)fx;
+        const int y1 = y0 + (y0 < Hp - 1), x1 = x0 + (x0 < Wp - 1);
+        tys[j] = fy - y0; txs[j] = fx - x0;
+        o00[j] = (y0 - cy0) * DP * Wp + x0; o01[j] = (y0 - cy0) * DP * Wp + x1;
+        o10[j] = (y1 - cy0) * DP * Wp + x0; o11[j] = (y1 - cy0) * DP * Wp + x1;
+    }
+    const V tx = L::pack(txs), ty = L::pack(tys);
+    V cz[DP];
+#pragma unroll
+    for (int k = 0; k < DP; ++k) {
+        float s00[P], s01[P], s10[P], s11[P];
+#pragma unroll
+        for (int j = 0; j < P; ++j) {
+            s00[j] = rows[k * Wp + o00[j]]; s01[j] = rows[k * Wp + o01[j]];
+            s10[j] = rows[k * Wp + o10[j]]; s11[j] = rows[k * Wp + o11[j]];
+        }
+        const V a = L::pack(s00) * (1.f - tx) + L::pack(s01) * tx;
+        const V bb = L::pack(s10) * (1.f - tx) + L::pack(s11) * tx;
+        cz[k] = a * (1.f - ty) + bb * ty;
+    }
+    constexpr float sd = D > 1 ? (float)(DP - 1) / (float)(D - 1) : 0.f;
+    V v[D];
+    V m = -INFINITY;
+#pragma unroll
+    for (int d = 0; d < D; ++d) {
+        const float fd = sd * (float)d;
+        const int k0 = (int)fd;
+        const int k1 = k0 + (k0 < DP - 1);
+        const float td = fd - (float)k0;
+        v[d] = cz[k0] * (1.f - td) + cz[k1] * td;
+        m = sa_max(m, v[d]);
+    }
+    V se = 0.f, sde = 0.f;
+#pragma unroll
+    for (int d = 0; d < D; ++d) {
+        const V e = sa_exp2((v[d] - m) * 1.44269504088896340736f);
+        se += e;
+        sde = sa_fma(e, (V)(float)(mindisp + d), sde);
+    }
+#pragma unroll
+    for (int j = 0; j < P; ++j) out[j] = L::lane(sde, j) / L::lane(se, j);
+}
+
+}
diff --git a/disprcnn_amd/csrc/disp_tail.hip b/disprcnn_amd/csrc/disp_tail.hip
--- /dev/null
+++ b/disprcnn_amd/csrc/disp_tail.hip
@@ -0,0 +1,110 @@
+#include <hip/hip_runtime.h>
+#include <stdint.h>
+
+#include "../../include/disprcnn_hip.h"
+#include "disp_tail.h"
+
+namespace {
+constexpr int kBand = DRC_DISP_TAIL_BAND;
+
+__host__ __device__ inline void band_rows(int band, int H, int Hp, float sy, int* cy0, int* cy1) {
+    const int ya = band * kBand;
+    const int yb = ya + kBand - 1 < H - 1 ? ya + kBand - 1 : H - 1;
+    *cy0 = (int)(sy * ya);
+    const int c1 = (int)(sy * yb) + 1;
+    *cy1 = c1 > Hp - 1 ? Hp - 1 : c1;
+}
+
+template <int DP, int D, int NH>
+__global__ __launch_bounds__(256) void disp_tail_planar_kernel(const HeadRows hr, const float* __restrict__ res, float* __restrict__ cost,
+                                                               float* __restrict__ disp, int Hp, int Wp, int H, int W, int mindisp, int bands,
+                                                               int maxrows) {
+    extern __shared__ float rows[];
+    int b = blockIdx.x;
+    if ((gridDim.x & 7) == 0) b = (b & 7) * (gridDim.x >> 3) + (b >> 3);
+    const int n = b / bands, band = b - n * bands;
+    const float sy = H > 1 ? (float)(Hp - 1) / (float)(H - 1) : 0.f;
+    const float sx = W > 1 ? (float)(Wp - 1) / (float)(W - 1) : 0.f;
+    int cy0, cy1;
+    band_rows(band, H, Hp, sy, &cy0, &cy1);
+    int nrows = cy1 - cy0 + 1;
+    nrows = nrows < maxrows ? nrows : maxrows;
+    const int span = nrows * Wp;
+    int own = Hp, unused;
+    if (band + 1 < bands) band_rows(band + 1, H, Hp, sy, &own, &unused);
+    for (int i = (int)threadIdx.x; i < DP * span; i += 256) {
+        const int k = i / span, rem = i - k * span;
+        const int r = rem / Wp, x = rem - r * Wp;
+        const int y = cy0 + r;
+        const long plane = (long)n * DP + k;
+        const float c0 = res ? res[(plane * Hp + y) * Wp + x] : 0.f;
+        const float c = head_planar_voxel<NH>(hr, c0, plane, y, x, Hp, Wp);
+        rows[(r * DP + k) * Wp + x] = c;
+        if (cost && y < own) cost[(plane * Hp + y) * Wp + x] = c;
+    }
+    __syncthreads();
+    const int pixa = band * kBand * W;
+    const int pixb = (band + 1) * kBand < H ? (band + 1) * kBand * W : H * W;
+    float* out = disp + (long)n * H * W;
+#pragma nounroll
+    for (int pix = pixa + (int)threadIdx.x; pix < pixb; pix += 256) {
+        float d;
+        softargmin_columns<DP, D, 1>(rows, cy0, Hp, Wp, W, sy, sx, &pix, mindisp, &d);
+        out[pix] = d;
+    }
+}
+
+template <int DP, int D>
+int launch(const HeadRows& hr, int nheads, const float* res, float* cost, float* disp, long blocks, int Hp, int Wp, int H, int W, int mindisp, int bands,
+           int maxrows, hipStream_t s) {
+    const dim3 g((unsigned)blocks), b(256);
+    const size_t lds = (size_t)maxrows * DP * Wp * sizeof(float);
+    if (nheads == 1) hipLaunchKernelGGL((disp_tail_planar_kernel<DP, D, 1>), g, b, lds, s, hr, res, cost, disp, Hp, Wp, H, W, mindisp, bands, maxrows);
+    else if (nheads == 2) hipLaunchKernelGGL((disp_tail_planar_kernel<DP, D, 2>), g, b, lds, s, hr, res, cost, disp, Hp, Wp, H, W, mindisp, bands, maxrows);
+    else hipLaunchKernelGGL((disp_tail_planar_kernel<DP, D, 3>), g, b, lds, s, hr, res, cost, disp, Hp, Wp, H, W, mindisp, bands, maxrows);
+    return (int)hipGetLastError();
+}
+}
+
+int drc_disp_tail_planar_rows(int Hp, int H, int* rows_sum) {
+    if (Hp <= 0 || H <= 0) return -2;
+    const float sy = H > 1 ? (float)(Hp - 1) / (float)(H - 1) : 0.f;
+    int most = 0, sum = 0;
+    for (int band = 0; band * kBand < H; ++band) {
+        int cy0, cy1;
+        band_rows(band, H, Hp, sy, &cy0, &cy1);
+        most = cy1 - cy0 + 1 > most ? cy1 - cy0 + 1 : most;
+        sum += cy1 - cy0 + 1;
+    }
+    if (rows_sum) *rows_sum = sum;
+    return most;
+}
+
+int drc_disp_tail_planar_form(int nheads, int Dp, int Hp, int Wp, int D, int H, int W) {
+    if (nheads < 1 || nheads > 3) return -2;
+    const int form = drc_upsample_softargmin_form(Dp, Hp, Wp, D, H, W);
+    if (form <= 0) return form;
+    if ((size_t)drc_disp_tail_planar_rows(Hp, H, nullptr) * Dp * Wp * sizeof(float) > 64 * 1024) return 0;
+    return form;
+}
+
+int drc_disp_tail_planar_fwd(const float* s0, const float* s1, const float* s2, float scale0, float scale1, float scale2, int nheads,
+                             const float* res, float* cost, float* disp, int N, int Dp, int Hp, int Wp, int D, int H, int W, int mindisp, void* stream) {
+    if (N < 0) return -2;
+    const int form = drc_disp_tail_planar_form(nheads, Dp, Hp, Wp, D, H, W);
+    if (form < 0) return form;
+    if (form == 0) return -4;
+    if (N == 0) return 0;
+    const HeadRows hr = {{s0, s1, s2}, {scale0, scale1, scale2}};
+    for (int k = 0; k < nheads; ++k)
+        if (!hr.rows[k] || ((uintptr_t)hr.rows[k] & 3)) return -1;
+    if (!disp) return -1;
+    const int bands = (H + kBand - 1) / kBand;
+    const long blocks = (long)N * bands;
+    if (blocks > 0x7fffffffL || (long)N * Dp * 9 * Hp * Wp > 0x7fffffffffffL) return -3;
+    const int maxrows = drc_disp_tail_planar_rows(Hp, H, nullptr);
+    hipStream_t s = (hipStream_t)stream;
+    if (form == 12) return launch<12, 48>(hr, nheads, res, cost, disp, blocks, Hp, Wp, H, W, mindisp, bands, maxrows, s);
+    if (form == 24) return launch<24, 96>(hr, nheads, res, cost, disp, blocks, Hp, Wp, H, W, mindisp, bands, maxrows, s);
+    return launch<6, 24>(hr, nheads, res, cost, disp, blocks, Hp, Wp, H, W, mindisp, bands, maxrows, s);
+}
diff --git a/disprcnn_amd/csrc/s16_ops.hip b/disprcnn_amd/csrc/s16_ops.hip
--- a/disprcnn_amd/csrc/s16_ops.hip
+++ b/disprcnn_amd/csrc/s16_ops.hip
@@ -3,6 +3,7 @@
 
 #include "../../include/disprcnn_hip.h"
 #include "s16_ovf.h"
+#include "disp_tail.h"
 
 typedef float f32x4 __attribute__((ext_vector_type(4)));
 typedef _Float16 f16x8 __attribute__((ext_vector_type(8)));
@@ -255,10 +256,6 @@
 }
 
 namespace {
-struct HeadRows {
-    const float* rows[3];
-    float scale[3];
-};
 template <int NH>
 __global__ __launch_bounds__(256) void head_gather_rows_kernel(const HeadRows hr, const float* __restrict__ res, float* __restrict__ cost, long cols, int H, int W) {
     typedef float f32x4 __attribute__((ext_vector_type(4)));
@@ -314,30 +311,7 @@
     const long plane = i / HW;
     const int e = (int)(i - plane * HW);
     const int y = e / W, x = e - y * W;
-    const bool xm = x > 0, xp = x + 1 < W, ym = y > 0, yp = y + 1 < H;
-    const int dm = xm ? -1 : 0, dp = xp ? 1 : 0, du = ym ? -W : 0, dd = yp ? W : 0;
-    float v[NH][9];
-#pragma unroll
-    for (int k = 0; k < NH; ++k) {
-        const float* p = hr.rows[k] + plane * 9 * HW + e;
-#pragma unroll
-        for (int j = 0; j < 9; ++j) v[k][j] = p[j * HW + (j < 3 ? du : j < 6 ? 0 : dd) + (j % 3 == 0 ? dm : j % 3 == 2 ? dp : 0)];
-    }
-    float c = res ? res[i] : 0.f;
-#pragma unroll
-    for (int k = 0; k < NH; ++k) {
-        const float* q = v[k];
-        const float l0 = xm ? q[0] : 0.f, l3 = xm ? q[3] : 0.f, l6 = xm ? q[6] : 0.f;
-        const float r2 = xp ? q[2] : 0.f, r5 = xp ? q[5] : 0.f, r8 = xp ? q[8] : 0.f;
-        const float t0 = (l0 + q[1]) + r2;
-        const float t1a = l3 + q[4];
-        const float t1b = r5;
-        const float t2 = (l6 + q[7]) + r8;
-        float s = (ym ? t0 : 0.f) + (t1a + t1b);
-        if (yp) s += t2;
-        c = hr.scale[k] * s + c;
-    }
-    cost[i] = c;
+    cost[i] = head_planar_voxel<NH>(hr, res ? res[i] : 0.f, plane, y, x, H, W);
 }
 }
 
diff --git a/disprcnn_amd/csrc/volume_ops.hip b/disprcnn_amd/csrc/volume_ops.hip
--- a/disprcnn_amd/csrc/volume_ops.hip
+++ b/disprcnn_amd/csrc/volume_ops.hip
@@ -2,6 +2,7 @@
 #include <stdint.h>
 
 #include "../../include/disprcnn_hip.h"
+#include "disp_tail.h"
 
 typedef float f32x4 __attribute__((ext_vector_type(4)));
 
@@ -393,9 +394,10 @@
     disp[idx] = sde / se;
 }
 
-template <int DP, int D>
-__global__ __launch_bounds__(256) void upsample_softargmin_t_kernel(const float* __restrict__ cost, float* __restrict__ disp, int N, int Hp, int Wp,
-                                                                    int H, int W, int mindisp, int blocks_per_roi) {
+template <int DP, int D, int P>
+__global__ __launch_bounds__(256 / P) void upsample_softargmin_t_kernel(const float* __restrict__ cost, float* __restrict__ disp, int N, int Hp,
+                                                                        int Wp, int H, int W, int mindisp, int blocks_per_roi) {
+    constexpr int T = 256 / P;
     extern __shared__ float rows[];
     int b = blockIdx.x;
     if ((gridDim.x & 7) == 0) b = (b & 7) * (gridDim.x >> 3) + (b >> 3);
@@ -411,56 +413,34 @@
     const int nrows = cy1 - cy0 + 1;
     const float* c = cost + (long)n * DP * Hp * Wp;
     const int lpr = Wp <= 32 ? 32 : 64, xl = (int)threadIdx.x & (lpr - 1);
-    for (int rk = (int)threadIdx.x / lpr; rk < nrows * DP; rk += 256 / lpr) {
+    for (int rk = (int)threadIdx.x / lpr; rk < nrows * DP; rk += T / lpr) {
         const int r = rk / DP, k = rk - r * DP;
         if (xl < Wp) rows[rk * Wp + xl] = c[((long)k * Hp + cy0 + r) * Wp + xl];
     }
     __syncthreads();
-    const int pix = pix0 + (int)threadIdx.x;
-    if (pix >= HW) return;
-    const int y = pix / W, x = pix - y * W;
-    const float fy = sy * y, fx = sx * x;
-    const int y0 = (int)fy, x0 = (int)fx;
-    const int y1 = y0 + (y0 < Hp - 1), x1 = x0 + (x0 < Wp - 1);
-    const float ty = fy - y0, tx = fx - x0;
-    const float* r0 = rows + (y0 - cy0) * DP * Wp;
-    const float* r1 = rows + (y1 - cy0) * DP * Wp;
-    float cz[DP];
-#pragma unroll
-    for (int k = 0; k < DP; ++k) {
-        const float a = r0[k * Wp + x0] * (1.f - tx) + r0[k * Wp + x1] * tx;
-        const float bb = r1[k * Wp + x0] * (1.f - tx) + r1[k * Wp + x1] * tx;
-        cz[k] = a * (1.f - ty) + bb * ty;
-    }
-    constexpr float sd = D > 1 ? (float)(DP - 1) / (float)(D - 1) : 0.f;
-    float v[D];
-    float m = -INFINITY;
-#pragma unroll
-    for (int d = 0; d < D; ++d) {
-        constexpr float dummy = 0.f; (void)dummy;
-        const float fd = sd * (float)d;
-        const int k0 = (int)fd;
-        const int k1 = k0 + (k0 < DP - 1);
-        const float td = fd - (float)k0;
-        v[d] = cz[k0] * (1.f - td) + cz[k1] * td;
-        m = fmaxf(m, v[d]);
-    }
-    float se = 0.f, sde = 0.f;
-#pragma unroll
-    for (int d = 0; d < D; ++d) {
-        const float e = __builtin_amdgcn_exp2f((v[d] - m) * 1.44269504088896340736f);
-        se += e;
-        sde = fmaf(e, (float)(mindisp + d), sde);
-    }
-    disp[(long)n * HW + pix] = sde / se;
+    int pix[P];
+#pragma unroll
+    for (int j = 0; j < P; ++j) pix[j] = pix0 + (int)threadIdx.x + j * T;
+    if (pix[0] >= HW) return;
+#pragma unroll
+    for (int j = 1; j < P; ++j) pix[j] = pix[j] < HW ? pix[j] : pl;
+    float out[P];
+    softargmin_columns<DP, D, P>(rows, cy0, Hp, Wp, W, sy, sx, pix, mindisp, out);
+    disp[(long)n * HW + pix[0]] = out[0];
+#pragma unroll
+    for (int j = 1; j < P; ++j)
+        if (pix0 + (int)threadIdx.x + j * T < HW) disp[(long)n * HW + pix[j]] = out[j];
 }
 
 template <int DP, int D>
-static int launch_softargmin_t(const float* cost, float* disp, int N, int Hp, int Wp, int H, int W, int mindisp, hipStream_t stream) {
+static int launch_softargmin_t(const float* cost, float* disp, int N, int Hp, int Wp, int H, int W, int mindisp, int packed, hipStream_t stream) {
     const int bpr = (H * W + 255) / 256;
     const long blocks = (long)N * bpr;
-    hipLaunchKernelGGL((upsample_softargmin_t_kernel<DP, D>), dim3((unsigned)blocks), dim3(256), (size_t)3 * DP * Wp * sizeof(float), stream, cost, disp, N,
-                       Hp, Wp, H, W, mindisp, bpr);
+    const size_t lds = (size_t)3 * DP * Wp * sizeof(float);
+    if (packed)
+        hipLaunchKernelGGL((upsample_softargmin_t_kernel<DP, D, 2>), dim3((unsigned)blocks), dim3(128), lds, stream, cost, disp, N, Hp, Wp, H, W, mindisp, bpr);
+    else
+        hipLaunchKernelGGL((upsample_softargmin_t_kernel<DP, D, 1>), dim3((unsigned)blocks), dim3(256), lds, stream, cost, disp, N, Hp, Wp, H, W, mindisp, bpr);
     return (int)hipGetLastError();
 }
 
@@ -700,6 +680,11 @@
 
 int drc_upsample_softargmin_fwd(const float* cost, float* disp, int N, int Dp, int Hp, int Wp, int D, int H, int W, int mindisp,
                                 void* stream) {
+    return drc_upsample_softargmin_fwd_sel(cost, disp, N, Dp, Hp, Wp, D, H, W, mindisp, 0, stream);
+}
+
+int drc_upsample_softargmin_fwd_sel(const float* cost, float* disp, int N, int Dp, int Hp, int Wp, int D, int H, int W, int mindisp,
+                                    int packed, void* stream) {
     if (N < 0) return -2;
     int form = drc_upsample_softargmin_form(Dp, Hp, Wp, D, H, W);
     if (form < 0) return form;
@@ -708,9 +693,9 @@
     if (!cost || !disp) return -1;
     if ((long)N * ((H * W + 255) / 256) >= (1L << 31)) form = 0;
     hipStream_t s = (hipStream_t)stream;
-    if (form == 12) return launch_softargmin_t<12, 48>(cost, disp, N, Hp, Wp, H, W, mindisp, s);
-    if (form == 24) return launch_softargmin_t<24, 96>(cost, disp, N, Hp, Wp, H, W, mindisp, s);
-    if (form == 6) return launch_softargmin_t<6, 24>(cost, disp, N, Hp, Wp, H, W, mindisp, s);
+    if (form == 12) return launch_softargmin_t<12, 48>(cost, disp, N, Hp, Wp, H, W, mindisp, packed, s);
+    if (form == 24) return launch_softargmin_t<24, 96>(cost, disp, N, Hp, Wp, H, W, mindisp, packed, s);
+    if (form == 6) return launch_softargmin_t<6, 24>(cost, disp, N, Hp, Wp, H, W, mindisp, packed, s);
     const unsigned blocks = (unsigned)((total + kSAThreads - 1) / kSAThreads);
     hipLaunchKernelGGL(upsample_softargmin_kernel, dim3(blocks), dim3(kSAThreads), (size_t)Dp * kSAThreads * 4, (hipStream_t)stream, cost, disp, N, Dp, Hp, Wp, D, H, W, mindisp);
     return done();
diff --git a/disprcnn_amd/engine.py b/disprcnn_amd/engine.py
--- a/disprcnn_amd/engine.py
+++ b/disprcnn_amd/engine.py
@@ -838,16 +838,56 @@
         raise ValueError("head_gather_planar: out / res = contiguous fp32 [N,D,H,W]")
     ptrs = [_ptr(r) for r in planes] + [None] * (3 - len(planes))
     sc = [C.c_float(float(s)) for s in scales] + [C.c_float(0.0)] * (3 - len(planes))
+    e0 = None if TIMING is None else _timing_start(out.device)
     st = _lib.lib().drc_head_gather_planar_fwd(ptrs[0], ptrs[1], ptrs[2], sc[0], sc[1], sc[2], len(planes), _ptr(res), _ptr(out), N, D, H, W, _stream_ptr(out.device))
     _lib.check(st, "drc_head_gather_planar_fwd")
+    if e0 is not None:
+        _timing_stop(e0, out.device, f"head_gather_planar_kernel<{len(planes)}>", 0)
+
+
+SOFTARGMIN_PACKED = {"enabled": False}
+DISP_TAIL_FUSED = {"enabled": True}
 
 
 def upsample_softargmin(cost, disp, maxdisp, mindisp):
     N, Dp, Hp, Wp = cost.shape
     _, H, W = disp.shape
-    st = _lib.lib().drc_upsample_softargmin_fwd(_ptr(cost), _ptr(disp), N, Dp, Hp, Wp, maxdisp - mindisp, H, W, mindisp,
-                                                _stream_ptr(cost.device))
+    e0 = None if TIMING is None else _timing_start(cost.device)
+    st = _lib.lib().drc_upsample_softargmin_fwd_sel(_ptr(cost), _ptr(disp), N, Dp, Hp, Wp, maxdisp - mindisp, H, W, mindisp,
+                                                    1 if SOFTARGMIN_PACKED["enabled"] else 0, _stream_ptr(cost.device))
     _lib.check(st, "drc_upsample_softargmin_fwd")
+    if e0 is not None:
+        form = _lib.lib().drc_upsample_softargmin_form(Dp, Hp, Wp, maxdisp - mindisp, H, W)
+        _timing_stop(e0, cost.device, f"upsample_softargmin_t_kernel<{form},{4 * form}>" if form > 0 else "upsample_softargmin_kernel", 0)
+
+
+def disp_tail_planar_form(nheads, Dp, Hp, Wp, D, H, W):
+    return _lib.lib().drc_disp_tail_planar_form(nheads, Dp, Hp, Wp, D, H, W)
+
+
+def disp_tail_planar(planes, scales, res, disp, maxdisp, mindisp, cost=None):
+    N, H, W = disp.shape
+    Dp = (maxdisp - mindisp) // 4
+    like = cost if cost is not None else res
+    Hp, Wp = (like.shape[2], like.shape[3]) if like is not None else (H // 4, W // 4)
+    if not 1 <= len(planes) <= 3 or len(scales) != len(planes):
+        raise ValueError("disp_tail_planar: 1 to 3 heads, one scale each")
+    for r in planes:
+        if r.dtype != torch.float32 or r.numel() < N * Dp * Hp * Wp * 9 or not r.is_contiguous():
+            raise ValueError("disp_tail_planar: planes = contiguous fp32 buffers of N*D'*9*H'*W'")
+    for t in (res, cost):
+        if t is not None and (t.dtype != torch.float32 or tuple(t.shape) != (N, Dp, Hp, Wp) or not t.is_contiguous()):
+            raise ValueError("disp_tail_planar: res / cost = contiguous fp32 [N,D',H',W']")
+    if disp.dtype != torch.float32 or not disp.is_contiguous():
+        raise ValueError("disp_tail_planar: disp = contiguous fp32 [N,H,W]")
+    ptrs = [_ptr(r) for r in planes] + [None] * (3 - len(planes))
+    sc = [C.c_float(float(s)) for s in scales] + [C.c_float(0.0)] * (3 - len(planes))
+    e0 = None if TIMING is None else _timing_start(disp.device)
+    st = _lib.lib().drc_disp_tail_planar_fwd(ptrs[0], ptrs[1], ptrs[2], sc[0], sc[1], sc[2], len(planes), _ptr(res), _ptr(cost), _ptr(disp), N, Dp, Hp, Wp,
+                                             maxdisp - mindisp, H, W, mindisp, _stream_ptr(disp.device))
+    _lib.check(st, "drc_disp_tail_planar_fwd")
+    if e0 is not None:
+        _timing_stop(e0, disp.device, f"disp_tail_planar_kernel<{Dp},{4 * Dp},{len(planes)}>", 0)
 
 
 def _geom8(t):
diff --git a/disprcnn_amd/modeling/psmnet/runtime.py b/disprcnn_amd/modeling/psmnet/runtime.py
--- a/disprcnn_amd/modeling/psmnet/runtime.py
+++ b/disprcnn_amd/modeling/psmnet/runtime.py
@@ -277,6 +277,8 @@
             planar = bool(ws["heads"][0][0][0].head_flat())
             for e, h in ws["heads"]:
                 run(*e, head=(h16[h.k][0], rows[h.k - 1]), head_layout=E.HEAD_PLANAR if planar else E.HEAD_ROWS_LAYOUT)
+            if planar and E.DISP_TAIL_FUSED["enabled"]:
+                return None, None, _PlanarTail([rows[0], rows[1], rows[2]], [h16[k][1] for k in (1, 2, 3)], t["costk3"])
             (E.head_gather_planar if planar else E.head_gather_rows)([rows[0], rows[1], rows[2]], [h16[k][1] for k in (1, 2, 3)], None, t["costk3"])
             return None, None, t["costk3"]
         for e, h in ws["heads"]:
@@ -288,6 +290,11 @@
                 E.conv3d_cout1(t[h.cls_t], W[h.weight], prev, t[h.costk])
             prev = t[h.costk]
         return t["costk1"], t["costk2"], t["costk3"]
+
+
+class _PlanarTail:
+    def __init__(self, planes, scales, cost):
+        self.planes, self.scales, self.cost = planes, scales, cost
 
 
 class PSMNetRuntime:
@@ -612,6 +619,14 @@
         outs = []
         for c in (costs if training else costs[2:]):
             d = torch.empty(N, H, W, dtype=torch.float32, device=self.device)
+            if isinstance(c, _PlanarTail):
+                Dp, Hp, Wp = c.cost.shape[1:]
+                if E.disp_tail_planar_form(len(c.planes), Dp, Hp, Wp, mx - mn, H, W) > 0:
+                    E.disp_tail_planar(c.planes, c.scales, None, d, mx, mn, cost=c.cost)
+                    outs.append(d)
+                    continue
+                E.head_gather_planar(c.planes, c.scales, None, c.cost)
+                c = c.cost
             E.upsample_softargmin(c, d, mx, mn)
             outs.append(d)
         return tuple(outs) if training else outs[0]
@@ -693,7 +708,7 @@
         m = self.model
         return (m.maxdisp, m.mindisp, getattr(m, "regressor_math", "auto"), getattr(m, "regressor_storage", "f32"),
                 getattr(m, "feature_storage", "f32"), getattr(m, "feature_math", "auto"),
-                E.S16["enabled"], E.HEAD_FUSED["enabled"], E.LASTCONV_S16["enabled"], E.TRUNK_S16["enabled"], E.CV_WIDE["enabled"], E.HEAD_ROWS["enabled"], tuple(sorted(E.HEAD_FLAT.items())), E.s16_allowed(),
+                E.S16["enabled"], E.HEAD_FUSED["enabled"], E.LASTCONV_S16["enabled"], E.TRUNK_S16["enabled"], E.CV_WIDE["enabled"], E.HEAD_ROWS["enabled"], tuple(sorted(E.HEAD_FLAT.items())), E.DISP_TAIL_FUSED["enabled"], E.s16_allowed(),
                 id(E.guard_in_scope()))
 
     def forward_features(self, fl, fr, out_hw, training=False):
diff --git a/include/disprcnn_hip.h b/include/disprcnn_hip.h
--- a/include/disprcnn_hip.h
+++ b/include/disprcnn_hip.h
@@ -110,6 +110,8 @@
 int drc_upsample_softargmin_fwd(const float* cost, float* disp, int N, int Dp, int Hp, int Wp,
                                 int D, int H, int W, int mindisp, void* stream);
 int drc_upsample_softargmin_form(int Dp, int Hp, int Wp, int D, int H, int W);
+int drc_upsample_softargmin_fwd_sel(const float* cost, float* disp, int N, int Dp, int Hp, int Wp,
+                                    int D, int H, int W, int mindisp, int packed, void* stream);
 
 int drc_pack_weights(const float* w, int cout, int cin, int K, int transposed, int flip, float* out_tap, float* out_t16, void* stream);
 
@@ -190,6 +192,12 @@
                              const float* res, float* cost, int N, int D, int H, int W, void* stream);
 int drc_head_gather_planar_fwd(const float* s0, const float* s1, const float* s2, float scale0, float scale1, float scale2, int nheads,
                                const float* res, float* cost, int N, int D, int H, int W, void* stream);
+#define DRC_DISP_TAIL_BAND 16
+int drc_disp_tail_planar_form(int nheads, int Dp, int Hp, int Wp, int D, int H, int W);
+int drc_disp_tail_planar_fwd(const float* s0, const float* s1, const float* s2, float scale0, float scale1, float scale2, int nheads,
+                             const float* res, float* cost, float* disp, int N, int Dp, int Hp, int Wp, int D, int H, int W, int mindisp,
+                             void* stream);
+int drc_disp_tail_planar_rows(int Hp, int H, int* rows_sum);
 int drc_conv3d_k3s2_s16_supported(int cin, int cout, int D, int H, int W);
 int drc_conv3d_k3s2_s16_fwd(const drc_s16conv_params* p, void* stream);
 int drc_deconv3d_k3s2_s16_supported(int cin, int cout, int D, int H, int W);
```

New measurement: 66770 ROI cost-volumes/s, median of 6. About the same (+0.9%).
